# nmonette/TO-UED

Hardware: NVIDIA B200
Metric: gridworld agent env-steps/sec incl. LPG update (higher is better)
Workload: dtype f16/bf16 operands, f32 accumulate (GRU); f32 elsewhere

## Files before the change

include/toued.h:

```cpp
#ifndef TOUED_H
#define TOUED_H
#include <stdint.h>
#ifdef __cplusplus
extern "C" {
#endif

#define TOUED_LEVEL_BYTES 192

const char* toued_last_error(void);
int toued_version(void);

int toued_rollout(const void* levels, const uint32_t* keys, const float* actor,
                  const uint8_t* forced_actions, int32_t* state, int32_t* obs, uint8_t* action,
                  float* reward, uint8_t* done, float* ep_return, int n_agents, int n_workers,
                  int rollout_len, int obs_dim, int max_grid_size, int max_n_objs, int reset_first,
                  void* stream);

int toued_env_step(const void* levels, const uint32_t* keys, const int32_t* actions, int32_t* state,
                   int32_t* obs, float* reward, uint8_t* done, int n_agents, int n_workers,
                   int max_grid_size, int max_n_objs, void* stream);
int toued_env_reset(const void* levels, int32_t* state, int32_t* obs, int n_agents, int n_workers,
                    int max_grid_size, void* stream);


int toued_sort_tokens(const int32_t* obs, uint16_t* sorted_tok, int n_agents, int n_workers,
                      int rollout_len, void* stream);

int toued_lpg_prepare(const int32_t* obs, const uint8_t* action, const float* reward,
                      const uint8_t* done, const float* actor, const float* critic,
                      const float* lpg_params, const int32_t* step, const void* levels, float* x,
                      void* ximg, int n_agents, int n_workers, int rollout_len, int obs_dim,
                      int lifetime_conditioning, int lpg_stride, void* stream);

int toued_gru_forward(const float* x, const uint8_t* done, const float* lpg_params, float* h_out,
                      float* gates, float* pi_hat, float* y_hat, int n_agents, int n_workers,
                      int rollout_len, int lifetime_conditioning, int lpg_stride, void* stream);

int toued_agent_scratch_floats(int n_agents, int n_workers, int rollout_len, int obs_dim);
int toued_agent_update(const int32_t* obs, const uint8_t* action, const uint16_t* sorted_tok,
                       const float* pi_hat, const float* y_hat, const float* actor_in,
                       const float* critic_in, float* actor_out, float* critic_out,
                       const void* levels, int32_t* step, float* scalars, int n_agents,
                       int n_workers, int rollout_len, int obs_dim, float lr_actor, float lr_critic,
                       float max_grad_norm, float agent_target_coeff, int tables_precopied, float* run_scratch,
                       void* stream);


int toued_meta_loss(const int32_t* obs, const uint8_t* action, const float* reward,
                    const uint8_t* done, const uint16_t* sorted_tok, const float* value_table,
                    const float* actor, float* lam, float* mu, float* scalars, int n_agents,
                    int n_workers, int rollout_len, int obs_dim, int value_stride, float gamma,
                    float gae_lambda, float grad_scale, int outer_product_quirk, void* stream);

int toued_agent_backward(const int32_t* obs, const uint8_t* action, const uint16_t* sorted_tok,
                         const float* pi_hat, const float* y_hat, const float* actor_k,
                         const float* critic_k, const float* actor_k1, const float* critic_k1,
                         const float* update_scalars, float* lam, float* mu, float* d_pi_hat,
                         float* d_y_hat, int n_agents, int n_workers, int rollout_len, int obs_dim,
                         float lr_actor, float lr_critic, float max_grad_norm,
                         float agent_target_coeff, float policy_entropy_coeff,
                         float target_entropy_coeff, float policy_l2_coeff, float target_l2_coeff,
                         float grad_scale, float* run_scratch, void* stream);

int toued_transpose_wh(const float* lpg_params, float* whT, void* stream);

int toued_gru_backward(const uint8_t* done, const float* lpg_params, const float* whT,
                       const float* h, float* gates, const float* y_hat, const float* d_pi_hat,
                       const float* d_y_hat, float* dl, float* dx, int n_agents, int n_workers,
                       int rollout_len, int lifetime_conditioning, void* stream);

int toued_lpg_wgrad_workspace_floats(void);
int toued_lpg_wgrad(const int32_t* obs, const uint8_t* done, const float* critic,
                    const float* lpg_params, const float* x, const float* h, const float* dgates,
                    const float* d_pi_hat, const float* dl, const float* dx, float* workspace,
                    int n_agents, int n_workers, int rollout_len, int obs_dim,
                    int lifetime_conditioning, int accumulate, void* stream);
int toued_lpg_wgrad_workspace_offset(int which);
int toued_lpg_wgrad_embed(const int32_t* obs, const uint8_t* done, const float* critic, const float* lpg_params,
                          const float* dx, float* workspace, const uint32_t* cotangent_max, int n_agents, int n_workers,
                          int rollout_len, int obs_dim, int lifetime_conditioning, int accumulate, void* stream);
int toued_lpg_wgrad_splits(int which);
int toued_reduce_partials(const float* workspace, float* grad, int lifetime_conditioning, int wh_splits,
                          int sm_splits, void* stream);

int toued_adam(float* params, const float* grad, float* mu, float* nu, int n, int count, float lr,
               float b1, float b2, float eps, void* stream);
int toued_adam_dev(float* params, const float* grad, float* mu, float* nu, int* count_dev, int n, float lr,
                   float b1, float b2, float eps, void* stream);
int toued_sgd_clip(float* params, const float* grad, float* sqnorm_scratch, int n, float lr, float max_norm,
                   void* stream);

int toued_a2c_update(const int32_t* obs, const uint8_t* action, const float* reward, const uint8_t* done,
                     const uint16_t* sorted_tok, const float* actor_in, const float* critic_in,
                     float* actor_out, float* critic_out, const void* levels, int32_t* step,
                     float* scalars, int n_agents, int n_workers, int rollout_len, int obs_dim,
                     float lr_actor, float lr_critic, float max_grad_norm, float gamma, float gae_lambda,
                     float entropy_coeff, int outer_product_quirk, void* stream);

int toued_a2c_train(const void* levels, const uint32_t* keys, float* actor0, float* actor1, float* critic0,
                    float* critic1, int32_t* state, int32_t* obs, uint8_t* action, float* reward, uint8_t* done,
                    uint16_t* sorted_tok, int32_t* step, float* scalars, float* loss_sums, int num_updates,
                    int n_agents, int n_workers, int rollout_len, int obs_dim, int max_grid_size, int max_n_objs,
                    float lr_actor, float lr_critic, float max_grad_norm, float gamma, float gae_lambda,
                    float entropy_coeff, int outer_product_quirk, void* stream);

int toued_es_ask(const uint32_t* key, const float* mean, float sigma, float* candidates, int popsize,
                 int n_params, int cand_stride, void* stream);
int toued_es_tell(const float* candidates, const float* fitness, float* mean, float* m, float* v,
                  int popsize, int n_params, int cand_stride, float sigma, float lrate, float beta1,
                  float beta2, float eps, int gen_counter, float mean_decay, void* stream);

int toued_es_ask_shard(const uint32_t* key, const float* mean, float sigma, float* candidates, int popsize_global,
                       int n_params, int cand_stride, int pair_offset, int n_pairs, void* stream);
int toued_es_grad_partial(const float* candidates, const float* fitness, const float* mean, float* grad_sum,
                          int n_members, int n_params, int cand_stride, float sigma, void* stream);
int toued_es_adam(const float* grad_sum, float* mean, float* m, float* v, int popsize_global, int n_params,
                  float sigma, float lrate, float beta1, float beta2, float eps, int gen_counter, float mean_decay,
                  void* stream);

int toued_plr_reset_lowest(float* score, uint8_t* active, uint8_t* is_new, int buffer_size, int minimum_new,
                           int* reset_ids, void* stream);
int toued_plr_select(uint32_t key0, uint32_t key1, float* score, uint8_t* active, uint8_t* is_new, int buffer_size,
                     const int* old_ids, const uint8_t* terminated, const float* new_scores, int n_agents,
                     float p_replay, float temperature, int shuffle_rounds, int* new_ids, void* stream);

int toued_generate_levels_desc_bytes(void);
int toued_generate_levels(const void* gen_desc, const uint32_t* keys, const int32_t* buffer_ids, void* levels_out,
                          int32_t* lifetimes_out, int n_levels, void* stream);

int toued_optimal_return(const void* levels, int n_levels, int horizon, int max_grid_size, int max_n_objs,
                         double* out, void* stream);

int toued_get_nash(const float* game, const float* x0, const float* y0, float* x_out, float* y_out,
                   int n, int x_nz, int y_nz, int num_iters, float lr, void* stream);
int toued_projection_simplex(float* v, int n, int max_nz, void* stream);


int toued_init_tables(const uint32_t* keys, const uint8_t* mask, float* tables, int n_agents,
                      int obs_dim, int n_out, void* stream);
int toued_masked_reset(const void* levels, const uint8_t* mask, int32_t* state, int32_t* obs,
                       int32_t* step, int n_agents, int n_workers, int max_grid_size, void* stream);

int toued_host_iota_bits(const uint32_t* keys, int n_keys, int n, uint32_t* out);


int toued_key_split(const uint32_t* keys_in, int n_keys, int num, int offset, int count, uint32_t* out,
                    void* stream);
int toued_key_chain(const uint32_t* keys_in, int n_keys, int chain_len, uint32_t* keys_out,
                    uint32_t* carry_out, void* stream);


int toued_tc_gemm_test(const float* A, const float* B, void* scratch_img, float* D, void* stream);
int toued_tc_gemm_mixed_test(const float* A, const float* B, void* scratch_img, float* D, void* stream);
int toued_tc_gemm_mn_test(const float* A, const float* B, void* scratch_img, float* D, int lbo, int sbo,
                          int kadv, void* stream);
int toued_tc_gemm_mn2_test(const float* A, const float* B, void* scratch_img, float* D, void* stream);

int toued_pack_wh_forward(const float* lpg_params, void* wh_img, int lifetime_conditioning, void* stream);
int toued_gru_forward_tc(const float* x, const uint8_t* done, const float* lpg_params, const void* wh_img,
                         void* h16, void* fac, void* hpimg, float* pi_hat, float* y_hat, int n_agents,
                         int n_workers, int rollout_len, int lifetime_conditioning, void* stream);
int toued_pack_wh_forward_multi(const float* lpg_params, void* wh_img, int lifetime_conditioning, int n_sets,
                                int lpg_stride, void* stream);
int toued_gru_forward_tc_multi(const float* x, const uint8_t* done, const float* lpg_params, const void* wh_img,
                               float* pi_hat, float* y_hat, int n_agents, int n_workers, int rollout_len,
                               int lifetime_conditioning, int lpg_stride, void* stream);

int toued_pack_wh_backward(const float* lpg_params, void* whb_img, void* stream);
#define TOUED_STATUS_NONFINITE_COT 1u
#define TOUED_STATUS_FP16_RANGE 2u
int toued_cotangent_max(const float* d_pi_hat, const float* d_y_hat, int n_agents, int n_workers, int rollout_len,
                        uint32_t* cotangent_max, void* stream);
int toued_gru_backward_tc(const uint8_t* done, const float* lpg_params, const void* whb_img,
                          const void* h16, const void* fac, const float* y_hat, const float* d_pi_hat,
                          const float* d_y_hat, void* dgimg, float* dl, float* dx, uint32_t* cotangent_max,
                          int n_agents, int n_workers, int rollout_len, int lifetime_conditioning, void* stream);
int toued_wgrad_tc_splits(void);
int toued_wgrad_tc_small_splits(void);
int toued_lpg_wgrad_tc(const void* hpimg, const void* dgimg, const void* ximg, const void* h16,
                       const float* d_pi_hat, const float* dl, float* wh_partials, float* small_partials,
                       uint32_t* cotangent_max, int n_agents, int n_workers, int rollout_len, int accumulate,
                       void* stream);

#ifdef __cplusplus
}
#endif
#endif
```

to_ued_b200/_lib.py:

```python
from __future__ import annotations

import ctypes as C
import os

_HERE = os.path.dirname(os.path.abspath(__file__))
_VARIANT = os.environ.get("TOUED_LIB_VARIANT", "")
LIB_PATH = os.path.join(_HERE, f"libtoued_{_VARIANT}.so" if _VARIANT else "libtoued.so")

_lib = None


class TouedError(RuntimeError):
    pass


def lib() -> C.CDLL:
    global _lib
    if _lib is None:
        if not os.path.exists(LIB_PATH):
            raise TouedError(
                f"{LIB_PATH} is missing: the CUDA extension is not built. "
                "Run `python -m to_ued_b200.csrc.build` (there is no CPU fallback).")
        _lib = C.CDLL(LIB_PATH)
        _declare(_lib)
    return _lib


_P, _I, _F = C.c_void_p, C.c_int, C.c_float

SIGNATURES = {
    "toued_rollout": [_P] * 10 + [_I] * 7 + [_P],
    "toued_env_step": [_P] * 7 + [_I] * 4 + [_P],
    "toued_env_reset": [_P] * 3 + [_I] * 3 + [_P],
    "toued_sort_tokens": [_P] * 2 + [_I] * 3 + [_P],
    "toued_lpg_prepare": [_P] * 11 + [_I] * 6 + [_P],
    "toued_gru_forward": [_P] * 7 + [_I] * 5 + [_P],
    "toued_agent_update": [_P] * 12 + [_I] * 4 + [_F] * 4 + [_I, _P, _P],
    "toued_agent_scratch_floats": [_I] * 4,
    "toued_meta_loss": [_P] * 10 + [_I] * 5 + [_F] * 3 + [_I, _P],
    "toued_agent_backward": [_P] * 14 + [_I] * 4 + [_F] * 9 + [_P, _P],
    "toued_transpose_wh": [_P] * 3,
    "toued_gru_backward": [_P] * 10 + [_I] * 4 + [_P],
    "toued_lpg_wgrad_workspace_floats": [],
    "toued_lpg_wgrad": [_P] * 11 + [_I] * 6 + [_P],
    "toued_reduce_partials": [_P, _P, _I, _I, _I, _P],
    "toued_lpg_wgrad_splits": [_I],
    "toued_lpg_wgrad_workspace_offset": [_I],
    "toued_lpg_wgrad_embed": [_P] * 7 + [_I] * 6 + [_P],
    "toued_cotangent_max": [_P, _P, _I, _I, _I, _P, _P],
    "toued_pack_wh_backward": [_P] * 3,
    "toued_gru_backward_tc": [_P] * 12 + [_I] * 4 + [_P],
    "toued_wgrad_tc_splits": [],
    "toued_wgrad_tc_small_splits": [],
    "toued_lpg_wgrad_tc": [_P] * 9 + [_I] * 4 + [_P],
    "toued_adam": [_P] * 4 + [_I, _I] + [_F] * 4 + [_P],
    "toued_adam_dev": [_P] * 5 + [_I] + [_F] * 4 + [_P],
    "toued_sgd_clip": [_P] * 3 + [_I, _F, _F, _P],
    "toued_get_nash": [_P] * 5 + [_I] * 4 + [_F, _P],
    "toued_projection_simplex": [_P, _I, _I, _P],
    "toued_es_ask": [_P, _P, _F, _P, _I, _I, _I, _P],
    "toued_es_tell": [_P] * 5 + [_I, _I, _I] + [_F] * 5 + [_I, _F, _P],
    "toued_es_ask_shard": [_P, _P, _F, _P, _I, _I, _I, _I, _I, _P],
    "toued_es_grad_partial": [_P] * 4 + [_I, _I, _I, _F, _P],
    "toued_es_adam": [_P] * 4 + [_I, _I] + [_F] * 5 + [_I, _F, _P],
    "toued_a2c_update": [_P] * 12 + [_I] * 4 + [_F] * 6 + [_I, _P],
    "toued_a2c_train": [_P] * 15 + [_I] * 7 + [_F] * 6 + [_I, _P],
    "toued_init_tables": [_P] * 3 + [_I] * 3 + [_P],
    "toued_masked_reset": [_P] * 5 + [_I] * 3 + [_P],
    "toued_generate_levels_desc_bytes": [],
    "toued_generate_levels": [_P] * 5 + [_I, _P],
    "toued_plr_reset_lowest": [_P] * 3 + [_I, _I, _P, _P],
    "toued_plr_select": [C.c_uint32, C.c_uint32] + [_P] * 3 + [_I] + [_P] * 3 + [_I, _F, _F, _I, _P, _P],
    "toued_tc_gemm_test": [_P] * 5,
    "toued_tc_gemm_mixed_test": [_P] * 5,
    "toued_tc_gemm_mn_test": [_P] * 4 + [_I] * 3 + [_P],
    "toued_tc_gemm_mn2_test": [_P] * 5,
    "toued_pack_wh_forward": [_P, _P, _I, _P],
    "toued_pack_wh_forward_multi": [_P, _P, _I, _I, _I, _P],
    "toued_gru_forward_tc_multi": [_P] * 6 + [_I] * 5 + [_P],
    "toued_host_iota_bits": [_P, _I, _I, _P],
    "toued_key_split": [_P, _I, _I, _I, _I, _P, _P],
    "toued_key_chain": [_P, _I, _I, _P, _P, _P],
    "toued_gru_forward_tc": [_P] * 9 + [_I] * 4 + [_P],
    "toued_optimal_return": [_P] + [_I] * 4 + [_P, _P],
}


def _declare(l):
    l.toued_last_error.restype = C.c_char_p
    l.toued_last_error.argtypes = []
    l.toued_version.restype = _I
    l.toued_version.argtypes = []
    for name, args in SIGNATURES.items():
        fn = getattr(l, name)
        fn.restype = _I
        fn.argtypes = args


def ptr(t):
    if t is None:
        return None
    if not t.is_cuda:
        raise TouedError("to_ued_b200 ops need CUDA tensors (there is no CPU fallback)")
    if not t.is_contiguous():
        raise TouedError("to_ued_b200 ops need contiguous tensors")
    return t.data_ptr()


def stream_ptr():
    import torch
    return torch.cuda.current_stream().cuda_stream


KERNELS_PER_CALL = {"toued_adam_dev": 2, "toued_sgd_clip": 2, "toued_lpg_wgrad": 3, "toued_init_tables": 2, "toued_lpg_wgrad_tc": 2, "toued_pack_wh_forward": 2, "toued_pack_wh_forward_multi": 2}
LAUNCHES = {}
GRAPH_KERNELS = [0]
ENV_STEPS = [0]
PROFILE = None


H2D_BYTES = [0]


def h2d(t):
    H2D_BYTES[0] += int(t.numel() * t.element_size()) if hasattr(t, "element_size") else int(t.nbytes)
    return t


def reset_counters(profile=False):
    global PROFILE
    H2D_BYTES[0] = 0
    GRAPH_KERNELS[0] = 0
    ENV_STEPS[0] = 0
    LAUNCHES.clear()
    PROFILE = {} if profile else None


def kernel_launches():
    return sum(n * KERNELS_PER_CALL.get(k, 1) for k, n in LAUNCHES.items()) + GRAPH_KERNELS[0]


def profile_ms():
    return {k: (len(v), sum(a.elapsed_time(b) for a, b in v)) for k, v in (PROFILE or {}).items()}


def call(name, *args):
    LAUNCHES[name] = LAUNCHES.get(name, 0) + 1
    if name == "toued_rollout":
        ENV_STEPS[0] += args[10] * args[11] * args[12]
    elif name == "toued_a2c_train":
        ENV_STEPS[0] += args[15] * args[16] * args[17] * args[18]
    if PROFILE is not None:
        import torch
        a, b = torch.cuda.Event(enable_timing=True), torch.cuda.Event(enable_timing=True)
        a.record()
        rc = getattr(lib(), name)(*args)
        b.record()
        PROFILE.setdefault(name, []).append((a, b))
    else:
        rc = getattr(lib(), name)(*args)
    if rc != 0:
        raise TouedError(f"{name} failed ({rc}): {lib().toued_last_error().decode()}")
```

to_ued_b200/agents/lpg_agent.py:

```python
from __future__ import annotations

from dataclasses import dataclass, field
from typing import Any, List, Optional

import numpy as np
import torch

from .. import _lib
from ..util import prng
from ..util.data import AgentState, Transition


@dataclass
class LPGAgentMetrics:
    policy_l2: Any
    policy_entropy: Any
    critic_loss: Any
    critic_l2: Any
    critic_entropy: Any

    def as_dict(self):
        return {"policy_l2": self.policy_l2, "policy_entropy": self.policy_entropy,
                "critic_loss": self.critic_loss, "critic_l2": self.critic_l2,
                "critic_entropy": self.critic_entropy}


class Tape:

    def __init__(self, n_agents, n_workers, rollout_len, obs_dim, num_updates, device, keep_gates=True,
                 precision=None, per_agent_params=False):
        import to_ued_b200
        N, W, L, D, K = n_agents, n_workers, rollout_len, obs_dim, num_updates
        R, dev = N * W, device
        f32, u8, i32 = torch.float32, torch.uint8, torch.int32
        self.N, self.W, self.L, self.D, self.K, self.R = N, W, L, D, K, R
        self.record = bool(keep_gates)
        kt = K + 1 if self.record else 2
        kr = K + 1 if self.record else 1
        ka = K if self.record else 1
        self.kt, self.kr, self.ka = kt, kr, ka
        self.actor = torch.empty((kt, N, D, 8), dtype=f32, device=dev)
        self.critic = torch.empty((kt, N, D, 8), dtype=f32, device=dev)
        self.obs = torch.empty((kr, N, L + 1, W), dtype=i32, device=dev)
        self.action = torch.empty((kr, N, L, W), dtype=u8, device=dev)
        self.reward = torch.empty((kr, N, L, W), dtype=f32, device=dev)
        self.done = torch.empty((kr, N, L, W), dtype=u8, device=dev)
        self.sorted_tok = torch.empty((kr, N, L * W), dtype=torch.int16, device=dev)
        self.precision = precision or to_ued_b200.GRU_PRECISION
        self.x = torch.empty((ka, L, R, 8), dtype=f32, device=dev)
        self.ximg = None
        if self.precision == "tc":
            f16 = torch.float16
            Rp = (R + 63) // 64 * 64
            R32 = (R + 31) // 32 * 32
            self.h16 = torch.empty((ka, L, R32, 256), dtype=f16, device=dev) if self.record and not per_agent_params else None
            self.fac = torch.empty((ka, 4, L, R32, 256), dtype=f16, device=dev) if self.record else None
            self.hpimg = torch.zeros((ka, L * Rp * 256 * 2), dtype=torch.uint8, device=dev) if self.record else None
            self.ximg = torch.zeros((ka, L * Rp * 128), dtype=torch.uint8, device=dev) if self.record else None
            self.wh_img = torch.zeros((N if per_agent_params else 1) * 16 * 26624 // 2, dtype=f16, device=dev)
            self.h = self.gates = None
        else:
            self.h = torch.empty((ka, L, R, 256), dtype=f32, device=dev)
            self.gates = torch.empty((ka, 4, L, R, 256), dtype=f32, device=dev) if self.record else None
        self.pi_hat = torch.empty((ka, L, R), dtype=f32, device=dev)
        self.y_hat = torch.empty((ka, L, R, 8), dtype=f32, device=dev)
        self.scalars = torch.empty((ka, N, 8), dtype=f32, device=dev)
        self.scal_sum = torch.zeros((N, 8), dtype=f32, device=dev)
        self.step_in = torch.empty((ka, N), dtype=i32, device=dev)
        self.ep_return = torch.empty((N, W), dtype=f32, device=dev)
        self.agent_scratch = torch.empty(_lib.lib().toued_agent_scratch_floats(N, W, L, D), dtype=f32, device=dev)

    def ti(self, k):
        return k if self.record else (k & 1)

    def ri(self, k):
        return k if self.record else 0

    def ai(self, k):
        return k if self.record else 0

    def transition(self, k) -> Transition:
        r = self.ri(k)
        return Transition(self.obs[r], self.action[r], self.reward[r], self.done[r])


_SORT_STREAMS = {}


def _sort_stream(cur):
    key = (cur.device.index, cur.cuda_stream)
    st = _SORT_STREAMS.get(key)
    if st is None:
        st = _SORT_STREAMS[key] = torch.cuda.Stream(device=cur.device)
    return st


def _mark(label):
    import to_ued_b200
    if to_ued_b200.PHASE_EVENTS is not None and getattr(to_ued_b200, "PHASE_FINE", False):
        e = torch.cuda.Event(enable_timing=True)
        e.record(torch.cuda.current_stream())
        to_ued_b200.PHASE_EVENTS.append((label, -2, e))


def lpg_agent_train_step(k, tape: Tape, levels, step, lpg_params, lifetime_conditioning, agent_target_coeff,
                         lr_actor, lr_critic, max_grad_norm, lpg_stride=0):
    N, W, L, D = tape.N, tape.W, tape.L, tape.D
    s = _lib.stream_ptr()
    p = _lib.ptr
    r, a, t0, t1 = tape.ri(k), tape.ai(k), tape.ti(k), tape.ti(k + 1)
    import to_ued_b200
    cur = torch.cuda.current_stream()
    side = _sort_stream(cur) if to_ued_b200.SIDE_STREAMS else cur
    ev_roll, ev_sort = torch.cuda.Event(), torch.cuda.Event()
    ev_roll.record(cur)
    with torch.cuda.stream(side):
        side.wait_event(ev_roll)
        _lib.call("toued_sort_tokens", p(tape.obs[r]), p(tape.sorted_tok[r]), N, W, L, _lib.stream_ptr())
        precopied = bool(to_ued_b200.SIDE_STREAMS)
        if precopied:
            tape.actor[t1].copy_(tape.actor[t0])
            tape.critic[t1].copy_(tape.critic[t0])
        ev_sort.record(side)
    _mark("rollout")
    tape.step_in[a].copy_(step)
    _lib.call("toued_lpg_prepare", p(tape.obs[r]), p(tape.action[r]), p(tape.reward[r]), p(tape.done[r]),
              p(tape.actor[t0]), p(tape.critic[t0]), p(lpg_params), p(step), p(levels), p(tape.x[a]),
              p(tape.ximg[a]) if tape.ximg is not None else None,
              N, W, L, D, int(lifetime_conditioning), int(lpg_stride), s)
    if lpg_stride and tape.precision == "tc":
        _lib.call("toued_gru_forward_tc_multi", p(tape.x[a]), p(tape.done[r]), p(lpg_params), p(tape.wh_img),
                  p(tape.pi_hat[a]), p(tape.y_hat[a]), N, W, L, int(lifetime_conditioning), int(lpg_stride), s)
    elif lpg_stride or tape.precision != "tc":
        _lib.call("toued_gru_forward", p(tape.x[a]), p(tape.done[r]), p(lpg_params), p(tape.h[a]),
                  p(tape.gates[a]) if tape.gates is not None else None, p(tape.pi_hat[a]), p(tape.y_hat[a]),
                  N, W, L, int(lifetime_conditioning), int(lpg_stride), s)
    else:
        _lib.call("toued_gru_forward_tc", p(tape.x[a]), p(tape.done[r]), p(lpg_params), p(tape.wh_img),
                  p(tape.h16[a]) if tape.h16 is not None else None, p(tape.fac[a]) if tape.fac is not None else None,
                  p(tape.hpimg[a]) if tape.hpimg is not None else None, p(tape.pi_hat[a]), p(tape.y_hat[a]),
                  N, W, L, int(lifetime_conditioning), s)
    _mark("gru_fwd")
    cur.wait_event(ev_sort)
    _mark("sort_wait")
    _lib.call("toued_agent_update", p(tape.obs[r]), p(tape.action[r]), p(tape.sorted_tok[r]), p(tape.pi_hat[a]),
              p(tape.y_hat[a]), p(tape.actor[t0]), p(tape.critic[t0]), p(tape.actor[t1]), p(tape.critic[t1]),
              p(levels), p(step), p(tape.scalars[a]), N, W, L, D, float(lr_actor), float(lr_critic),
              float(max_grad_norm), float(agent_target_coeff), int(precopied), p(tape.agent_scratch), s)
    tape.scal_sum += tape.scalars[a]
    _mark("update")


def train_lpg_agent_steps(rng, lpg_train_state, agent_state: AgentState, rollout_manager, num_train_steps: int,
                          agent_target_coeff: float, tape: Optional[Tape] = None, lpg_stride: int = 0):
    env = rollout_manager.env
    actor, critic = agent_state.actor_state, agent_state.critic_state
    N, W = agent_state.env_state.packed.shape
    L, K = rollout_manager.train_rollout_len, num_train_steps
    dev = actor.params.device
    if tape is None:
        import to_ued_b200
        tape = Tape(N, W, L, env.obs_dim, K, dev, keep_gates=False,
                    precision=to_ued_b200.ES_PRECISION if lpg_stride else None, per_agent_params=bool(lpg_stride))
    levels = agent_state.level.packed
    step = actor.step.clone()
    state = agent_state.env_state.packed.clone()
    tape.actor[0].copy_(actor.params)
    tape.critic[0].copy_(critic.params)
    tape.scal_sum.zero_()
    keys_d = prng.chain_device(prng.to_device(rng, dev), K)
    p = _lib.ptr
    lpg = lpg_train_state.params if hasattr(lpg_train_state, "params") else lpg_train_state
    cond = lpg_train_state.model.lifetime_conditioning if hasattr(lpg_train_state, "model") else False
    if tape.precision == "tc" and not lpg_stride:
        _lib.call("toued_pack_wh_forward", p(lpg), p(tape.wh_img), int(cond), _lib.stream_ptr())
    elif tape.precision == "tc":
        _lib.call("toued_pack_wh_forward_multi", p(lpg), p(tape.wh_img), int(cond), N, int(lpg_stride), _lib.stream_ptr())
    yield
    for k in range(K):
        r = tape.ri(k)
        _lib.call("toued_rollout", p(levels), p(keys_d[k]), p(tape.actor[tape.ti(k)]), None, p(state), p(tape.obs[r]),
                  p(tape.action[r]), p(tape.reward[r]), p(tape.done[r]), None, N, W, L, env.obs_dim,
                  env.max_grid_size, env.max_n_objs, 0, _lib.stream_ptr())
        lpg_agent_train_step(k, tape, levels, step, lpg, cond, agent_target_coeff, actor.learning_rate,
                             critic.learning_rate, actor.max_grad_norm, lpg_stride=lpg_stride)
        yield
    sc = tape.scal_sum / K
    metrics = LPGAgentMetrics(policy_l2=sc[:, 4], policy_entropy=sc[:, 6], critic_loss=sc[:, 3],
                              critic_l2=sc[:, 5], critic_entropy=sc[:, 7])
    from ..environments.gridworld.gridworld import EnvState
    new_agent = agent_state.replace(
        actor_state=actor.replace(params=tape.actor[tape.ti(K)].clone(), step=step),
        critic_state=critic.replace(params=tape.critic[tape.ti(K)].clone(), step=step.clone()),
        env_obs=tape.obs[tape.ri(K - 1)][:, -1].clone(), env_state=EnvState(state, env.max_n_objs))
    rollouts = [tape.transition(k) for k in range(K)] if tape.record else [tape.transition(K - 1)]
    return new_agent, rollouts, metrics


def train_lpg_agent(rng, lpg_train_state, agent_state: AgentState, rollout_manager, num_train_steps: int,
                    agent_target_coeff: float, tape: Optional[Tape] = None, lpg_stride: int = 0):
    gen = train_lpg_agent_steps(rng, lpg_train_state, agent_state, rollout_manager, num_train_steps,
                                agent_target_coeff, tape=tape, lpg_stride=lpg_stride)
    while True:
        try:
            next(gen)
        except StopIteration as done:
            return done.value
```

to_ued_b200/csrc/agent_backward.cu:

```cuda
#include "lpg_common.cuh"
#include "segreduce.cuh"
#include "../../include/toued.h"

__global__ void __launch_bounds__(256)
meta_loss_kernel(const int32_t* __restrict__ obs, const uint8_t* __restrict__ action,
                 const float* __restrict__ reward, const uint8_t* __restrict__ done,
                 const uint16_t* __restrict__ sorted_tok, const float* __restrict__ value,
                 const float* __restrict__ actor, float* __restrict__ lam, float* __restrict__ mu,
                 float* __restrict__ scal, int W, int L, int D, int vstride, float gamma, float lmbda,
                 float gscale, int quirk) {
    extern __shared__ __align__(16) float sm[];
    float* adv = sm;
    float* rec = adv + L * W;
    float* abar = rec + L * W * 6;
    float* lbar = abar + W;
    float* runv = lbar + W;
    float* scan = runv + L * W * 5;
    void* idxmem = scan + 2 * 256 * 5;
    __shared__ float red[32];
    __shared__ int iscan[512];
    __shared__ unsigned char sflags[512];
    const int n = blockIdx.x, tid = threadIdx.x, T = W * L;
    const int32_t* ob = obs + (size_t)n * (L + 1) * W;
    const uint8_t* act = action + (size_t)n * T;
    const float* rw = reward + (size_t)n * T;
    const uint8_t* dn = done + (size_t)n * T;
    const uint16_t* st = sorted_tok + (size_t)n * T;
    const float* vt = value + (size_t)n * D * vstride;
    const float* at = actor + (size_t)n * D * 8;
    float* lm = lam + (size_t)n * D * 8;
    float* mm = mu + (size_t)n * D * 8;
    const float invT = 1.0f / (float)T;
    const SegIndex si = seg_index_build(idxmem, iscan, st, ob, T);

    for (int i = tid; i < D * 2; i += 256) {
        reinterpret_cast<float4*>(lm)[i] = make_float4(0.f, 0.f, 0.f, 0.f);
        reinterpret_cast<float4*>(mm)[i] = make_float4(0.f, 0.f, 0.f, 0.f);
    }
    float s1 = 0.f, s2 = 0.f;
    const float vlast = vt[(size_t)(D - 1) * vstride];
    for (int w = tid; w < W; w += 256) {
        float g = 0.f;
        int32_t o1 = ob[L * W + w];
        float v1 = vt[(size_t)ob_idx(o1) * vstride] + 0.001f * (float)ob_time(o1) * vlast;
        for (int t = L - 1; t >= 0; --t) {
            const int32_t o0 = ob[t * W + w];
            const float v0 = vt[(size_t)ob_idx(o0) * vstride] + 0.001f * (float)ob_time(o0) * vlast;
            const float nd = dn[t * W + w] ? 0.0f : 1.0f;
            const float delta = rw[t * W + w] + gamma * v1 * nd - v0;
            g = delta + gamma * lmbda * nd * g;
            adv[t * W + w] = g;
            s1 += g; s2 = fmaf(g, g, s2);
            v1 = v0;
        }
    }
    s1 = block_sum(s1, red); s2 = block_sum(s2, red);
    const float mean = s1 * invT;
    float var = 0.f;
    for (int i = tid; i < T; i += 256) { const float d = adv[i] - mean; var = fmaf(d, d, var); }
    var = block_sum(var, red) * invT;
    const float inv_std = 1.0f / (sqrtf(var) + 1e-8f);
    __syncthreads();
    for (int i = tid; i < T; i += 256) adv[i] = (adv[i] - mean) * inv_std;
    __syncthreads();
    for (int tok = tid; tok < T; tok += 256) {
        const int32_t o = ob[tok];
        float z[5], p[5];
        tab_logits8<5>(at, D, o, z);
        softmax_c<5>(z, p);
        const int a = act[tok];
        float pa = p[0];
#pragma unroll
        for (int j = 1; j < 5; ++j) pa = (a == j) ? p[j] : pa;
        float* r = rec + tok * 6;
        r[5] = logf(pa + 1e-8f);
        const float q = pa / (pa + 1e-8f);
#pragma unroll
        for (int j = 0; j < 5; ++j) r[j] = q * ((a == j ? 1.0f : 0.0f) - p[j]);
    }
    __syncthreads();
    float loss = 0.f;
    for (int w = tid; w < W; w += 256) {
        float sa = 0.f, sl = 0.f, se = 0.f;
        for (int t = 0; t < L; ++t) { sa += adv[t * W + w]; sl += rec[(t * W + w) * 6 + 5]; se = fmaf(adv[t * W + w], rec[(t * W + w) * 6 + 5], se); }
        abar[w] = sa / (float)L; lbar[w] = sl / (float)L;
        loss -= quirk ? abar[w] * lbar[w] : se / (float)L;
    }
    loss = block_sum(loss, red) / (float)W;
    __syncthreads();
    float last[5] = {0.f, 0.f, 0.f, 0.f, 0.f};
    for (int tok = tid; tok < T; tok += 256) {
        const int w = tok % W;
        const float coef = -gscale * invT * (quirk ? abar[w] : adv[tok]);
        float* r = rec + tok * 6;
        const float tf = 0.001f * (float)ob_time(ob[tok]);
#pragma unroll
        for (int j = 0; j < 5; ++j) { r[j] *= coef; last[j] = fmaf(tf, r[j], last[j]); }
        r[5] = tf;
    }
#pragma unroll
    for (int j = 0; j < 5; ++j) last[j] = block_sum(last[j], red);
    __syncthreads();
    seg_reduce<5, 6>(rec, si, T, runv, scan, sflags);
    for (int r = tid; r < si.nruns; r += 256) {
        const int row = si.run_row[r];
#pragma unroll
        for (int j = 0; j < 5; ++j) lm[(size_t)row * 8 + j] = runv[r * 5 + j];
    }
    if (tid == 0) {
#pragma unroll
        for (int j = 0; j < 5; ++j) lm[(size_t)(D - 1) * 8 + j] = last[j];
        scal[n * 2 + 0] = loss;
        scal[n * 2 + 1] = s2 * invT;
    }
}

extern "C" int toued_meta_loss(const int32_t* obs, const uint8_t* action, const float* reward,
                               const uint8_t* done, const uint16_t* sorted_tok, const float* value_table,
                               const float* actor, float* lam, float* mu, float* scalars, int n_agents,
                               int n_workers, int rollout_len, int obs_dim, int value_stride, float gamma,
                               float gae_lambda, float grad_scale, int outer_product_quirk, void* stream) {
    const int T = n_workers * rollout_len;
    TOUED_CHECK(n_agents > 0 && T > 0, "toued_meta_loss: empty problem");
    const size_t smem = sizeof(float) * ((size_t)T * 7 + 2 * n_workers + (size_t)T * 5 + 2 * 256 * 5) + seg_index_bytes(T);
    TOUED_CHECK(smem <= 200 * 1024, "toued_meta_loss: W*L=%d too large for shared memory", T);
    TOUED_CUDA(cudaFuncSetAttribute(meta_loss_kernel, cudaFuncAttributeMaxDynamicSharedMemorySize, (int)smem));
    meta_loss_kernel<<<n_agents, 256, smem, (cudaStream_t)stream>>>(
        obs, action, reward, done, sorted_tok, value_table, actor, lam, mu, scalars, n_workers, rollout_len,
        obs_dim, value_stride, gamma, gae_lambda, grad_scale, outer_product_quirk);
    TOUED_LAUNCH_CHECK();
    return 0;
}

struct TokFwd { float p[5], y[8], pa, q, tf; int a; };

__device__ __forceinline__ TokFwd tok_forward(const float* at, const float* ct, int D, int32_t o, int a) {
    TokFwd f;
    float z[5], zy[8];
    tab_logits8<5>(at, D, o, z);
    softmax_c<5>(z, f.p);
    tab_logits8<8>(ct, D, o, zy);
    softmax_c<8>(zy, f.y);
    f.a = a;
    f.pa = f.p[0];
#pragma unroll
    for (int j = 1; j < 5; ++j) f.pa = (a == j) ? f.p[j] : f.pa;
    f.q = f.pa / (f.pa + 1e-8f);
    f.tf = 0.001f * (float)ob_time(o);
    return f;
}

__device__ __forceinline__ void tok_grad(const TokFwd& f, float ph, const float* yh, float invT, float alpha, float* c) {
    const float ca = invT * ph * f.q;
#pragma unroll
    for (int j = 0; j < 5; ++j) c[j] = ca * ((f.a == j ? 1.0f : 0.0f) - f.p[j]);
    float mm[8], b = 0.f;
#pragma unroll
    for (int i = 0; i < 8; ++i) {
        mm[i] = logf(f.y[i] + 1e-8f) - logf(yh[i] + 1e-8f) + f.y[i] / (f.y[i] + 1e-8f);
        b = fmaf(f.y[i], mm[i], b);
    }
    const float cc = alpha * invT;
#pragma unroll
    for (int i = 0; i < 8; ++i) c[5 + i] = cc * f.y[i] * (mm[i] - b);
}

__device__ __forceinline__ void load8(const float* p, float* v) {
    const float4 a = reinterpret_cast<const float4*>(p)[0], b = reinterpret_cast<const float4*>(p)[1];
    v[0] = a.x; v[1] = a.y; v[2] = a.z; v[3] = a.w; v[4] = b.x; v[5] = b.y; v[6] = b.z; v[7] = b.w;
}

__global__ void __launch_bounds__(256, 2)
agent_backward_kernel(const int32_t* __restrict__ obs, const uint8_t* __restrict__ action,
                      const uint16_t* __restrict__ sorted_tok, const float* __restrict__ pi_hat,
                      const float* __restrict__ y_hat, const float* __restrict__ actor_k,
                      const float* __restrict__ critic_k, const float* __restrict__ actor_k1,
                      const float* __restrict__ critic_k1, const float* __restrict__ upd_scal,
                      float* lam, float* mu, float* __restrict__ d_pi_hat, float* __restrict__ d_y_hat,
                      float* run_scratch, int n_agents, int W, int L, int D, float lr_a, float lr_c, float max_norm,
                      float alpha, float b_pent, float b_yent, float b_pl2, float b_yl2, float gscale) {
    extern __shared__ __align__(16) float rec[];
    __shared__ float red[32];
    __shared__ float s_wlast[13];
    __shared__ int iscan[512];
    __shared__ unsigned char sflags[512];
    const int n = blockIdx.x, tid = threadIdx.x, T = W * L, R = n_agents * W;
    const int32_t* ob = obs + (size_t)n * (L + 1) * W;
    const uint8_t* act = action + (size_t)n * T;
    const uint16_t* st = sorted_tok + (size_t)n * T;
    const float* a0 = actor_k + (size_t)n * D * 8;
    const float* c0 = critic_k + (size_t)n * D * 8;
    const float* a1 = actor_k1 + (size_t)n * D * 8;
    const float* c1 = critic_k1 + (size_t)n * D * 8;
    float* lm = lam + (size_t)n * D * 8;
    float* mm = mu + (size_t)n * D * 8;
    const float invT = 1.0f / (float)T;
    const float gna = upd_scal[n * 8 + 0], gnc = upd_scal[n * 8 + 1];
    const bool keep = upd_scal[n * 8 + 2] != 0.0f;
    float* runv = run_scratch + (size_t)n * min(T, D) * 13;
    float* scan = rec + (size_t)T * 13;
    const SegIndex si = seg_index_build(scan + 2 * 256 * 13, iscan, st, ob, T);

    float last[13];
#pragma unroll
    for (int j = 0; j < 13; ++j) last[j] = 0.f;
    for (int tok = tid; tok < T; tok += 256) {
        const TokFwd f = tok_forward(a1, c1, D, ob[tok], act[tok]);
        float* r = rec + tok * 13;
        {
            float dh[5], s = 0.f;
#pragma unroll
            for (int j = 0; j < 5; ++j) { dh[j] = -(logf(f.p[j] + 1e-8f) + 1.0f); s = fmaf(f.p[j], dh[j], s); }
            const float k = -b_pent * gscale * invT;
#pragma unroll
            for (int j = 0; j < 5; ++j) r[j] = k * f.p[j] * (dh[j] - s);
        }
        {
            float dh[8], s = 0.f;
#pragma unroll
            for (int j = 0; j < 8; ++j) { dh[j] = -(logf(f.y[j] + 1e-8f) + 1.0f); s = fmaf(f.y[j], dh[j], s); }
            const float k = -b_yent * gscale * invT;
#pragma unroll
            for (int j = 0; j < 8; ++j) r[5 + j] = k * f.y[j] * (dh[j] - s);
        }
#pragma unroll
        for (int j = 0; j < 13; ++j) last[j] = fmaf(f.tf, r[j], last[j]);
    }
#pragma unroll
    for (int j = 0; j < 13; ++j) last[j] = block_sum(last[j], red);
    __syncthreads();
    seg_reduce<13, 13>(rec, si, T, runv, scan, sflags);
    for (int r = tid; r < si.nruns; r += 256) {
        const int row = si.run_row[r];
        const float* g = runv + r * 13;
#pragma unroll
        for (int j = 0; j < 5; ++j) lm[(size_t)row * 8 + j] += g[j];
#pragma unroll
        for (int j = 0; j < 8; ++j) mm[(size_t)row * 8 + j] += g[5 + j];
    }
    if (tid == 0) {
#pragma unroll
        for (int j = 0; j < 5; ++j) lm[(size_t)(D - 1) * 8 + j] += last[j];
#pragma unroll
        for (int j = 0; j < 8; ++j) mm[(size_t)(D - 1) * 8 + j] += last[5 + j];
    }
    __syncthreads();

    const float dir_pi = gscale * b_pl2 * 2.0f * invT;
    const float dir_y = gscale * b_yl2 * 2.0f * invT;
    if (!keep) {
        for (int tok = tid; tok < T; tok += 256) {
            const int t = tok / W, w = tok - t * W;
            const size_t li = (size_t)t * R + (size_t)n * W + w;
            d_pi_hat[li] = dir_pi * pi_hat[li];
            float yh[8]; load8(y_hat + li * 8, yh);
            float4* o = reinterpret_cast<float4*>(d_y_hat + li * 8);
            o[0] = make_float4(dir_y * yh[0], dir_y * yh[1], dir_y * yh[2], dir_y * yh[3]);
            o[1] = make_float4(dir_y * yh[4], dir_y * yh[5], dir_y * yh[6], dir_y * yh[7]);
        }
        return;
    }

#pragma unroll
    for (int j = 0; j < 13; ++j) last[j] = 0.f;
    for (int tok = tid; tok < T; tok += 256) {
        const int t = tok / W, w = tok - t * W;
        const size_t li = (size_t)t * R + (size_t)n * W + w;
        const TokFwd f = tok_forward(a0, c0, D, ob[tok], act[tok]);
        float yh[8]; load8(y_hat + li * 8, yh);
        float* r = rec + tok * 13;
        tok_grad(f, pi_hat[li], yh, invT, alpha, r);
#pragma unroll
        for (int j = 0; j < 13; ++j) last[j] = fmaf(f.tf, r[j], last[j]);
    }
#pragma unroll
    for (int j = 0; j < 13; ++j) last[j] = block_sum(last[j], red);
    __syncthreads();
    seg_reduce<13, 13>(rec, si, T, runv, scan, sflags);
    float dot_a = 0.f, dot_c = 0.f;
    for (int r = tid; r < si.nruns; r += 256) {
        const int row = si.run_row[r];
        const float* g = runv + r * 13;
        float l8[8], m8[8];
        load8(lm + (size_t)row * 8, l8); load8(mm + (size_t)row * 8, m8);
#pragma unroll
        for (int j = 0; j < 5; ++j) dot_a = fmaf(g[j], l8[j], dot_a);
#pragma unroll
        for (int j = 0; j < 8; ++j) dot_c = fmaf(g[5 + j], m8[j], dot_c);
    }
    dot_a = block_sum(dot_a, red); dot_c = block_sum(dot_c, red);
    float ll[8], ml[8];
    load8(lm + (size_t)(D - 1) * 8, ll); load8(mm + (size_t)(D - 1) * 8, ml);
#pragma unroll
    for (int j = 0; j < 5; ++j) dot_a = fmaf(last[j], ll[j], dot_a);
#pragma unroll
    for (int j = 0; j < 8; ++j) dot_c = fmaf(last[5 + j], ml[j], dot_c);
    const bool clip_a = !(gna < max_norm), clip_c = !(gnc < max_norm);
    const float ka = -lr_a * (clip_a ? max_norm / gna : 1.0f), pa_ = clip_a ? dot_a / (gna * gna) : 0.0f;
    const float kc = -lr_c * (clip_c ? max_norm / gnc : 1.0f), pc_ = clip_c ? dot_c / (gnc * gnc) : 0.0f;
    if (tid == 0) {
#pragma unroll
        for (int j = 0; j < 5; ++j) s_wlast[j] = ka * (ll[j] - pa_ * last[j]);
#pragma unroll
        for (int j = 0; j < 8; ++j) s_wlast[5 + j] = kc * (ml[j] - pc_ * last[5 + j]);
    }
    __syncthreads();
    float wl[13];
#pragma unroll
    for (int j = 0; j < 13; ++j) wl[j] = s_wlast[j];

    for (int r = tid; r < si.nruns; r += 256) {
        const int row = si.run_row[r];
        float* g = runv + r * 13;
        float l8[8], m8[8];
        load8(lm + (size_t)row * 8, l8); load8(mm + (size_t)row * 8, m8);
#pragma unroll
        for (int j = 0; j < 5; ++j) g[j] = ka * (l8[j] - pa_ * g[j]);
#pragma unroll
        for (int j = 0; j < 8; ++j) g[5 + j] = kc * (m8[j] - pc_ * g[5 + j]);
    }
    __syncthreads();
    float hl[13];
#pragma unroll
    for (int j = 0; j < 13; ++j) hl[j] = 0.f;
    for (int pos = tid; pos < T; pos += 256) {
        const int tok = si.tok[pos];
        const int t = tok / W, w = tok - t * W;
        const size_t li = (size_t)t * R + (size_t)n * W + w;
        const TokFwd f = tok_forward(a0, c0, D, ob[tok], act[tok]);
        const float ph = pi_hat[li];
        float yh[8]; load8(y_hat + li * 8, yh);
        float* r = rec + tok * 13;
        const float* wr = runv + (size_t)si.run[pos] * 13;
        float v[13];
#pragma unroll
        for (int j = 0; j < 13; ++j) v[j] = fmaf(f.tf, wl[j], wr[j]);
        float va = v[0], pv = 0.f;
#pragma unroll
        for (int j = 1; j < 5; ++j) va = (f.a == j) ? v[j] : va;
#pragma unroll
        for (int j = 0; j < 5; ++j) pv = fmaf(f.p[j], v[j], pv);
        const float s = va - pv;
        d_pi_hat[li] = invT * f.q * s + dir_pi * ph;
        const float pe = f.pa + 1e-8f;
        const float c1_ = ph * invT * s * 1e-8f * f.pa / (pe * pe), c2_ = ph * invT * f.q;
        float h[13];
#pragma unroll
        for (int j = 0; j < 5; ++j)
            h[j] = c1_ * ((f.a == j ? 1.0f : 0.0f) - f.p[j]) - c2_ * f.p[j] * (v[j] - pv);
        float m[8], mp[8], av = 0.f, b = 0.f;
#pragma unroll
        for (int j = 0; j < 8; ++j) {
            const float ye = f.y[j] + 1e-8f;
            m[j] = logf(ye) - logf(yh[j] + 1e-8f) + f.y[j] / ye;
            mp[j] = (f.y[j] + 2e-8f) / (ye * ye);
            av = fmaf(v[5 + j], f.y[j], av);
            b = fmaf(f.y[j], m[j], b);
        }
        const float ca = alpha * invT;
        float dS[8], sy = 0.f, dyo[8];
#pragma unroll
        for (int j = 0; j < 8; ++j) {
            const float vc = v[5 + j];
            dyo[j] = ca * f.y[j] * (av - vc) / (yh[j] + 1e-8f) + dir_y * yh[j];
            dS[j] = vc * m[j] + vc * f.y[j] * mp[j] - vc * b - av * (m[j] + f.y[j] * mp[j]);
            sy = fmaf(f.y[j], dS[j], sy);
        }
#pragma unroll
        for (int j = 0; j < 8; ++j) h[5 + j] = ca * f.y[j] * (dS[j] - sy);
        float4* o = reinterpret_cast<float4*>(d_y_hat + li * 8);
        o[0] = make_float4(dyo[0], dyo[1], dyo[2], dyo[3]);
        o[1] = make_float4(dyo[4], dyo[5], dyo[6], dyo[7]);
#pragma unroll
        for (int j = 0; j < 13; ++j) { r[j] = h[j]; hl[j] = fmaf(f.tf, h[j], hl[j]); }
    }
#pragma unroll
    for (int j = 0; j < 13; ++j) hl[j] = block_sum(hl[j], red);
    __syncthreads();
    seg_reduce<13, 13>(rec, si, T, runv, scan, sflags);
    for (int r = tid; r < si.nruns; r += 256) {
        const int row = si.run_row[r];
        const float* g = runv + r * 13;
#pragma unroll
        for (int j = 0; j < 5; ++j) lm[(size_t)row * 8 + j] += g[j];
#pragma unroll
        for (int j = 0; j < 8; ++j) mm[(size_t)row * 8 + j] += g[5 + j];
    }
    if (tid == 0) {
#pragma unroll
        for (int j = 0; j < 5; ++j) lm[(size_t)(D - 1) * 8 + j] = ll[j] + hl[j];
#pragma unroll
        for (int j = 0; j < 8; ++j) mm[(size_t)(D - 1) * 8 + j] = ml[j] + hl[5 + j];
    }
}

extern "C" int toued_agent_backward(const int32_t* obs, const uint8_t* action, const uint16_t* sorted_tok,
                                    const float* pi_hat, const float* y_hat, const float* actor_k,
                                    const float* critic_k, const float* actor_k1, const float* critic_k1,
                                    const float* update_scalars, float* lam, float* mu, float* d_pi_hat,
                                    float* d_y_hat, int n_agents, int n_workers, int rollout_len, int obs_dim,
                                    float lr_actor, float lr_critic, float max_grad_norm,
                                    float agent_target_coeff, float policy_entropy_coeff,
                                    float target_entropy_coeff, float policy_l2_coeff, float target_l2_coeff,
                                    float grad_scale, float* run_scratch, void* stream) {
    const int T = n_workers * rollout_len;
    TOUED_CHECK(n_agents > 0 && T > 0, "toued_agent_backward: empty problem");
    TOUED_CHECK(run_scratch != nullptr, "toued_agent_backward: run_scratch (toued_agent_scratch_floats) is required");
    const size_t smem = sizeof(float) * ((size_t)T * 13 + 2 * 256 * 13) + seg_index_bytes(T);
    TOUED_CHECK(smem <= 200 * 1024, "toued_agent_backward: W*L=%d too large for shared memory", T);
    TOUED_CUDA(cudaFuncSetAttribute(agent_backward_kernel, cudaFuncAttributeMaxDynamicSharedMemorySize, (int)smem));
    TOUED_CUDA(cudaFuncSetAttribute(agent_backward_kernel, cudaFuncAttributePreferredSharedMemoryCarveout, 100));
    cudaStream_t st = (cudaStream_t)stream;
    agent_backward_kernel<<<n_agents, 256, smem, st>>>(
        obs, action, sorted_tok, pi_hat, y_hat, actor_k, critic_k, actor_k1, critic_k1, update_scalars, lam, mu,
        d_pi_hat, d_y_hat, run_scratch, n_agents, n_workers, rollout_len, obs_dim, lr_actor, lr_critic, max_grad_norm,
        agent_target_coeff, policy_entropy_coeff, target_entropy_coeff, policy_l2_coeff, target_l2_coeff, grad_scale);
    TOUED_LAUNCH_CHECK();
    return 0;
}
```

to_ued_b200/csrc/agent_update.cu:

```cuda
#include "lpg_common.cuh"
#include "segreduce.cuh"
#include "../../include/toued.h"

constexpr int AU_C = 13;

__global__ void __launch_bounds__(256, 2)
agent_update_kernel(const int32_t* __restrict__ obs, const uint8_t* __restrict__ action,
                    const uint16_t* __restrict__ sorted_tok, const float* __restrict__ pi_hat,
                    const float* __restrict__ y_hat, const float* __restrict__ actor_in,
                    const float* __restrict__ critic_in, float* actor_out, float* critic_out,
                    const LevelRec* __restrict__ levels, int32_t* __restrict__ step,
                    float* __restrict__ scal, float* run_scratch, int n_agents, int W, int L, int D,
                    float lr_a, float lr_c, float max_norm, float alpha, int tables_precopied) {
    extern __shared__ __align__(16) float smc[];
    __shared__ float red[32];
    __shared__ int iscan[512];
    __shared__ unsigned char sflags[512];
    const int n = blockIdx.x, tid = threadIdx.x, T = W * L, R = n_agents * W;
    float* runv = run_scratch + (size_t)n * min(T, D) * 13;
    float* scan = smc + (size_t)T * AU_C;
    void* idxmem = scan + 2 * 256 * 13;
    const int32_t* ob = obs + (size_t)n * (L + 1) * W;
    const uint8_t* act = action + (size_t)n * T;
    const float* a_in = actor_in + (size_t)n * D * 8;
    const float* c_in = critic_in + (size_t)n * D * 8;
    float* a_out = actor_out + (size_t)n * D * 8;
    float* c_out = critic_out + (size_t)n * D * 8;
    const float invT = 1.0f / (float)T;
    const SegIndex si = seg_index_build(idxmem, iscan, sorted_tok + (size_t)n * T, ob, T);

    if (!tables_precopied)
        for (int i = tid; i < D * 2; i += 256) {
            reinterpret_cast<float4*>(a_out)[i] = reinterpret_cast<const float4*>(a_in)[i];
            reinterpret_cast<float4*>(c_out)[i] = reinterpret_cast<const float4*>(c_in)[i];
        }

    float m_kl = 0.f, m_pi2 = 0.f, m_y2 = 0.f;
    float last[13];
#pragma unroll
    for (int j = 0; j < 13; ++j) last[j] = 0.f;
    for (int tok = tid; tok < T; tok += 256) {
        const int t = tok / W, w = tok - t * W;
        const size_t li = (size_t)t * R + (size_t)n * W + w;
        const int32_t o = ob[tok];
        float z[5], p[5], zy[8], y[8];
        tab_logits8<5>(a_in, D, o, z);
        softmax_c<5>(z, p);
        tab_logits8<8>(c_in, D, o, zy);
        softmax_c<8>(zy, y);
        const int a = act[tok];
        float pa = p[0];
#pragma unroll
        for (int j = 1; j < 5; ++j) pa = (a == j) ? p[j] : pa;
        const float ph = pi_hat[li];
        const float ca = invT * ph * (pa / (pa + 1e-8f));
        float* rec = smc + tok * AU_C;
#pragma unroll
        for (int j = 0; j < 5; ++j) rec[j] = ca * ((a == j ? 1.0f : 0.0f) - p[j]);
        float yh[8];
        { const float4* q = reinterpret_cast<const float4*>(y_hat + li * 8); const float4 q0 = q[0], q1 = q[1];
          yh[0] = q0.x; yh[1] = q0.y; yh[2] = q0.z; yh[3] = q0.w; yh[4] = q1.x; yh[5] = q1.y; yh[6] = q1.z; yh[7] = q1.w; }
        float mm[8], b = 0.f, kl = 0.f, y2 = 0.f;
#pragma unroll
        for (int i = 0; i < 8; ++i) {
            const float ly = logf(y[i] + 1e-8f), lh = logf(yh[i] + 1e-8f);
            mm[i] = ly - lh + y[i] / (y[i] + 1e-8f);
            b = fmaf(y[i], mm[i], b);
            kl = fmaf(y[i], ly - lh, kl);
            y2 = fmaf(yh[i], yh[i], y2);
        }
        const float cc = alpha * invT;
#pragma unroll
        for (int i = 0; i < 8; ++i) rec[5 + i] = cc * y[i] * (mm[i] - b);
        const float tf = 0.001f * (float)ob_time(o);
#pragma unroll
        for (int j = 0; j < 13; ++j) last[j] = fmaf(tf, rec[j], last[j]);
        m_kl += kl; m_pi2 = fmaf(ph, ph, m_pi2); m_y2 += y2;
    }
#pragma unroll
    for (int j = 0; j < 13; ++j) last[j] = block_sum(last[j], red);
    m_kl = block_sum(m_kl, red); m_pi2 = block_sum(m_pi2, red); m_y2 = block_sum(m_y2, red);
    __syncthreads();

    seg_reduce<13, AU_C>(smc, si, T, runv, scan, sflags);
    float na = 0.f, nc = 0.f;
    for (int r = tid; r < si.nruns; r += 256) {
        const float* g = runv + r * 13;
#pragma unroll
        for (int j = 0; j < 5; ++j) na = fmaf(g[j], g[j], na);
#pragma unroll
        for (int j = 5; j < 13; ++j) nc = fmaf(g[j], g[j], nc);
    }
    na = block_sum(na, red); nc = block_sum(nc, red);
#pragma unroll
    for (int j = 0; j < 5; ++j) na = fmaf(last[j], last[j], na);
#pragma unroll
    for (int j = 5; j < 13; ++j) nc = fmaf(last[j], last[j], nc);
    const float gna = sqrtf(na), gnc = sqrtf(nc);
    const float sa = gna < max_norm ? 1.0f : max_norm / gna;
    const float sc = gnc < max_norm ? 1.0f : max_norm / gnc;
    const int old_step = step[n];
    const bool keep = (old_step + 1) <= levels[n].lifetime;
    const float ua = keep ? lr_a * sa : 0.0f, uc = keep ? lr_c * sc : 0.0f;

    for (int r = tid; r < si.nruns; r += 256) {
        const int row = si.run_row[r];
        const float* g = runv + r * 13;
#pragma unroll
        for (int j = 0; j < 5; ++j) a_out[(size_t)row * 8 + j] = a_in[(size_t)row * 8 + j] - ua * g[j];
#pragma unroll
        for (int j = 0; j < 8; ++j) c_out[(size_t)row * 8 + j] = c_in[(size_t)row * 8 + j] - uc * g[5 + j];
    }
    if (tid == 0) {
#pragma unroll
        for (int j = 0; j < 5; ++j) a_out[(size_t)(D - 1) * 8 + j] = a_in[(size_t)(D - 1) * 8 + j] - ua * last[j];
#pragma unroll
        for (int j = 0; j < 8; ++j) c_out[(size_t)(D - 1) * 8 + j] = c_in[(size_t)(D - 1) * 8 + j] - uc * last[5 + j];
        step[n] = keep ? old_step + 1 : old_step;
    }
    __syncthreads();

    float ea = 0.f, ec = 0.f;
    for (int tok = tid; tok < T; tok += 256) {
        const int32_t o = ob[tok];
        float z[5], p[5], zy[8], y[8];
        tab_logits8<5>(a_out, D, o, z);
        softmax_c<5>(z, p);
        tab_logits8<8>(c_out, D, o, zy);
        softmax_c<8>(zy, y);
#pragma unroll
        for (int j = 0; j < 5; ++j) { const float q = p[j] + 1e-8f; ea -= q * logf(q); }
#pragma unroll
        for (int j = 0; j < 8; ++j) { const float q = y[j] + 1e-8f; ec -= q * logf(q); }
    }
    ea = block_sum(ea, red); ec = block_sum(ec, red);
    if (tid == 0) {
        float* s = scal + (size_t)n * 8;
        s[0] = gna; s[1] = gnc; s[2] = keep ? 1.0f : 0.0f;
        s[3] = m_kl * invT;
        s[4] = m_pi2 * invT;
        s[5] = m_y2 * invT;
        s[6] = ea * invT;
        s[7] = ec * invT;
    }
}

static size_t agent_smem_bytes(int T, int D) {
    return sizeof(float) * ((size_t)T * AU_C + 2 * 256 * 13) + seg_index_bytes(T);
}

extern "C" int toued_agent_update(const int32_t* obs, const uint8_t* action, const uint16_t* sorted_tok,
                                  const float* pi_hat, const float* y_hat, const float* actor_in,
                                  const float* critic_in, float* actor_out, float* critic_out,
                                  const void* levels, int32_t* step, float* scalars, int n_agents,
                                  int n_workers, int rollout_len, int obs_dim, float lr_actor,
                                  float lr_critic, float max_grad_norm, float agent_target_coeff, int tables_precopied,
                                  float* run_scratch, void* stream) {
    const int T = n_workers * rollout_len;
    const size_t smem = agent_smem_bytes(T, obs_dim);
    TOUED_CHECK(n_agents > 0 && T > 0, "toued_agent_update: empty problem");
    TOUED_CHECK(smem <= 200 * 1024, "toued_agent_update: W*L=%d too large for shared memory", T);
    TOUED_CHECK(actor_in != actor_out && critic_in != critic_out, "toued_agent_update: in-place update not supported");
    TOUED_CUDA(cudaFuncSetAttribute(agent_update_kernel, cudaFuncAttributeMaxDynamicSharedMemorySize, (int)smem));
    TOUED_CUDA(cudaFuncSetAttribute(agent_update_kernel, cudaFuncAttributePreferredSharedMemoryCarveout, 100));
    TOUED_CHECK(run_scratch != nullptr, "toued_agent_update: run_scratch (toued_agent_scratch_floats) is required");
    cudaStream_t st = (cudaStream_t)stream;
    agent_update_kernel<<<n_agents, 256, smem, st>>>(
        obs, action, sorted_tok, pi_hat, y_hat, actor_in, critic_in, actor_out, critic_out,
        (const LevelRec*)levels, step, scalars, run_scratch, n_agents, n_workers, rollout_len, obs_dim,
        lr_actor, lr_critic, max_grad_norm, agent_target_coeff, tables_precopied);
    TOUED_LAUNCH_CHECK();
    return 0;
}

extern "C" int toued_agent_scratch_floats(int n_agents, int n_workers, int rollout_len, int obs_dim) {
    const long long T = (long long)n_workers * rollout_len;
    const long long n = 13ll * (T < obs_dim ? T : obs_dim) * n_agents;
    return n < (1ll << 31) ? (int)n : -1;
}
```

to_ued_b200/csrc/lpg_common.cuh:

```cuda
#pragma once
#include "common.cuh"

constexpr int LPG_H = 256;
constexpr int LPG_Y = 8;
constexpr int LPG_E = 16;
constexpr int LPG_G = 3 * LPG_H;
constexpr int LPG_XP = 8;

struct LpgOffsets {
    int e_w0, e_b0, e_w1, e_b1, Wi, bi, Wh, bhn, w_pi, b_pi, W_y, b_y, total;
};
__host__ __device__ inline LpgOffsets lpg_offsets(int X) {
    LpgOffsets o; int p = 0;
    o.Wh = p; p += LPG_H * LPG_G;
    o.Wi = p; p += X * LPG_G;
    o.bi = p; p += LPG_G;
    o.bhn = p; p += LPG_H;
    o.w_pi = p; p += LPG_H;
    o.W_y = p; p += LPG_H * LPG_Y;
    o.b_y = p; p += LPG_Y;
    o.e_w0 = p; p += LPG_Y * LPG_E;
    o.e_b0 = p; p += LPG_E;
    o.e_w1 = p; p += LPG_E;
    o.e_b1 = p; p += 1;
    o.b_pi = p; p += 1;
    o.total = p;
    return o;
}

__device__ __forceinline__ float sigmoidf_(float x) { return 1.0f / (1.0f + __expf(-x)); }
__device__ __forceinline__ float tanhf_(float x) {
    const float e = __expf(2.0f * x);
    return 1.0f - 2.0f / (e + 1.0f);
}

__device__ __forceinline__ float ex2_approx(float x) { float y; asm("ex2.approx.ftz.f32 %0, %1;" : "=f"(y) : "f"(x)); return y; }
__device__ __forceinline__ float rcp_approx(float x) { float y; asm("rcp.approx.ftz.f32 %0, %1;" : "=f"(y) : "f"(x)); return y; }
__device__ __forceinline__ float tanh_mufu(float x) { float y; asm("tanh.approx.f32 %0, %1;" : "=f"(y) : "f"(x)); return y; }
__device__ __forceinline__ float sigmoid_mufu(float x) { return fmaf(0.5f, tanh_mufu(0.5f * x), 0.5f); }
__device__ __forceinline__ float sigmoid_fast(float x) { return rcp_approx(1.0f + ex2_approx(-1.4426950408889634f * x)); }
__device__ __forceinline__ float tanh_fast(float x) { return fmaf(2.0f, rcp_approx(1.0f + ex2_approx(-2.8853900817779268f * x)), -1.0f); }

__device__ __forceinline__ float fmin_nan(float a, float b) { float r; asm("min.NaN.f32 %0, %1, %2;" : "=f"(r) : "f"(a), "f"(b)); return r; }
__device__ __forceinline__ float fmax_nan(float a, float b) { float r; asm("max.NaN.f32 %0, %1, %2;" : "=f"(r) : "f"(a), "f"(b)); return r; }
__device__ __forceinline__ float fmax3_nan(float a, float b, float c) {
    float r; asm("max.NaN.f32 %0, %1, %2, %3;" : "=f"(r) : "f"(a), "f"(b), "f"(c)); return r;
}

template <int C>
__device__ __forceinline__ void softmax_c(const float (&z)[C], float (&p)[C]) {
    float m = z[0];
#pragma unroll
    for (int j = 1; j < C; ++j) m = fmaxf(m, z[j]);
    float s = 0.0f;
#pragma unroll
    for (int j = 0; j < C; ++j) { p[j] = __expf(z[j] - m); s += p[j]; }
    const float inv = 1.0f / s;
#pragma unroll
    for (int j = 0; j < C; ++j) p[j] *= inv;
}

template <int C>
__device__ __forceinline__ void tab_logits8(const float* table, int D, int32_t ob, float (&z)[C]) {
    const float tf = 0.001f * (float)ob_time(ob);
    const float4* row = reinterpret_cast<const float4*>(table + (size_t)ob_idx(ob) * 8);
    const float4* last = reinterpret_cast<const float4*>(table + (size_t)(D - 1) * 8);
    float r[8], l[8];
    const float4 a0 = row[0], a1 = row[1], b0 = last[0], b1 = last[1];
    r[0] = a0.x; r[1] = a0.y; r[2] = a0.z; r[3] = a0.w; r[4] = a1.x; r[5] = a1.y; r[6] = a1.z; r[7] = a1.w;
    l[0] = b0.x; l[1] = b0.y; l[2] = b0.z; l[3] = b0.w; l[4] = b1.x; l[5] = b1.y; l[6] = b1.z; l[7] = b1.w;
#pragma unroll
    for (int j = 0; j < C; ++j) z[j] = r[j] + tf * l[j];
}

__device__ __forceinline__ float block_sum(float v, float* red) {
#pragma unroll
    for (int o = 16; o > 0; o >>= 1) v += __shfl_xor_sync(0xffffffffu, v, o);
    const int lane = threadIdx.x & 31, warp = threadIdx.x >> 5, nw = (blockDim.x + 31) >> 5;
    __syncthreads();
    if (lane == 0) red[warp] = v;
    __syncthreads();
    float t = (lane < nw) ? red[lane] : 0.0f;
#pragma unroll
    for (int o = 16; o > 0; o >>= 1) t += __shfl_xor_sync(0xffffffffu, t, o);
    return t;
}
```

to_ued_b200/meta/train.py:

```python
from __future__ import annotations

from typing import Any, Optional

import numpy as np
import torch

from .. import _lib
from ..util import prng
from ..util.data import AgentState, LpgHyperparams
from ..agents.lpg_agent import Tape, train_lpg_agent, train_lpg_agent_steps
from ..agents.agents import eval_agent
from ..environments.gridworld.gridworld import EnvState


class LPGTrainState:

    def __init__(self, model, params, tx, opt_state=None, step=0):
        self.model, self.params, self.tx = model, params, tx
        self.opt_state = tx.init(params) if opt_state is None else opt_state
        self.step = step

    def replace(self, **kw):
        d = dict(model=self.model, params=self.params, tx=self.tx, opt_state=self.opt_state, step=self.step)
        d.update(kw)
        return LPGTrainState(**d)


class MetaGradWorkspace:

    def __init__(self, n_agents, n_workers, rollout_len, obs_dim, num_updates, n_params, device):
        N, W, L, K = n_agents, n_workers, rollout_len, num_updates
        R = N * W
        f32 = torch.float32
        self.tape = Tape(N, W, L, obs_dim, K, device, keep_gates=True)
        self.d_pi_hat2 = [torch.empty((L, R), dtype=f32, device=device) for _ in range(2)]
        self.d_y_hat2 = [torch.empty((L, R, 8), dtype=f32, device=device) for _ in range(2)]
        self.dx2 = [torch.empty((L, R, 2), dtype=f32, device=device) for _ in range(2)]
        self.d_pi_hat, self.d_y_hat, self.dx = self.d_pi_hat2[0], self.d_y_hat2[0], self.dx2[0]
        self.dl2 = [torch.empty((L, R, 8), dtype=f32, device=device) for _ in range(2)]
        self.dl = self.dl2[0]
        self.lam = torch.empty((N, obs_dim, 8), dtype=f32, device=device)
        self.mu = torch.empty((N, obs_dim, 8), dtype=f32, device=device)
        self.whT = torch.empty((768, 256), dtype=f32, device=device)
        self.partials = torch.empty(_lib.lib().toued_lpg_wgrad_workspace_floats(), dtype=f32, device=device)
        self.loss_scal = torch.empty((N, 2), dtype=f32, device=device)
        self.ab_scratch = torch.empty(_lib.lib().toued_agent_scratch_floats(N, W, L, obs_dim), dtype=f32, device=device)
        if self.tape.precision == "tc":
            Rp = (R + 63) // 64 * 64
            self.whb_img = torch.empty(256 * 768, dtype=torch.float16, device=device)
            self.cotmax = torch.zeros((K, 2), dtype=torch.int32, device=device)
            self.dgimg2 = [torch.zeros(L * Rp * 1024 * 2, dtype=torch.uint8, device=device) for _ in range(2)]
            self.dgimg = self.dgimg2[0]
        self.off_small = _lib.lib().toued_lpg_wgrad_workspace_offset(1)
        self.key = (N, W, L, obs_dim, K, n_params, str(device))


_WS_CACHE = {}
_STREAMS = {}


def _workspace(n, w, L, D, K, P, device, slot=0) -> MetaGradWorkspace:
    import to_ued_b200
    key = (n, w, L, D, K, P, str(device), to_ued_b200.GRU_PRECISION)
    if _WS_CACHE and next(iter(_WS_CACHE))[:-1] != key:
        _WS_CACHE.clear()
    ws = _WS_CACHE.get(key + (slot,))
    if ws is None:
        ws = _WS_CACHE[key + (slot,)] = MetaGradWorkspace(n, w, L, D, K, P, device)
    return ws


def reverse_status(reset=False):
    st = torch.zeros((), dtype=torch.int32, device="cuda")
    for ws in _WS_CACHE.values():
        if getattr(ws, "cotmax", None) is not None:
            for w in ws.cotmax[:, 1]:
                st = st | w
            if reset:
                ws.cotmax[:, 1].zero_()
    return st


def _eval_stream(device):
    key = ("eval", str(device))
    if key not in _STREAMS:
        _STREAMS[key] = [torch.cuda.Stream(device=device)]
    return _STREAMS[key][0]


def _side_streams(device, n):
    key = str(device)
    lst = _STREAMS.setdefault(key, [])
    while len(lst) < n:
        lst.append(torch.cuda.Stream(device=device))
    return lst[:n]


def _world():
    import torch.distributed as dist
    if dist.is_available() and dist.is_initialized():
        return dist.get_world_size(), dist
    return 1, None


def lpg_meta_grad_train_step(rng, lpg_train_state: LPGTrainState, agent_states: AgentState, value_critic_states,
                             rollout_manager, num_mini_batches: int, gamma: float, gae_lambda: float,
                             lpg_hypers: LpgHyperparams, *, outer_product_quirk: bool = True,
                             global_agent_offset: int = 0, global_num_agents: Optional[int] = None,
                             eval_workers: int = 4, return_grad: bool = False, num_streams: Optional[int] = None,
                             _static: Optional[dict] = None):
    env = rollout_manager.env
    actor, critic = agent_states.actor_state, agent_states.critic_state
    N, W = agent_states.env_state.packed.shape
    L, K, D = rollout_manager.train_rollout_len, lpg_hypers.num_agent_updates, env.obs_dim
    dev = actor.params.device
    world, dist = _world()
    n_global = global_num_agents if global_num_agents is not None else N * world
    if dist is not None and global_num_agents is None:
        global_agent_offset = dist.get_rank() * N
    model = lpg_train_state.model
    cond = int(model.lifetime_conditioning)
    lpg = lpg_train_state.params
    P = lpg.numel()
    p, s = _lib.ptr, _lib.stream_ptr()

    rngs = prng.split_device(prng.to_device(rng, dev), n_global, global_agent_offset, N)[0]
    r_train, r_eval, r_evalagent = prng.chain_device(rngs, 3)

    if N % num_mini_batches != 0:
        raise ValueError(f"local agents ({N}) must be divisible by num_mini_batches ({num_mini_batches})")
    nb = N // num_mini_batches
    import to_ued_b200
    if num_streams is None:
        num_streams = to_ued_b200.NUM_STREAMS
    S = max(1, min(int(num_streams), num_mini_batches))
    wss = [_workspace(nb, W, L, D, K, P, dev, slot=i) for i in range(S)]
    main = torch.cuda.current_stream()
    streams = [main] if S == 1 else _side_streams(dev, S)
    tc = wss[0].tape.precision == "tc"
    gscale = 1.0 / n_global
    bK = [c / K for c in (lpg_hypers.policy_entropy_coeff, lpg_hypers.target_entropy_coeff,
                          lpg_hypers.policy_l2_coeff, lpg_hypers.target_l2_coeff)]
    if _static is not None:
        new_actor, new_critic, new_step, new_state, new_obs = _static["out"]
    else:
        new_actor = torch.empty_like(actor.params)
        new_critic = torch.empty_like(critic.params)
        new_step = torch.empty_like(actor.step)
        new_state = torch.empty_like(agent_states.env_state.packed)
        new_obs = torch.empty_like(agent_states.env_obs)
    msums = [torch.zeros(8, dtype=torch.float32, device=dev) for _ in range(S)]
    returns = torch.empty(N, dtype=torch.float32, device=dev)
    ready = torch.cuda.Event()
    ready.record(main)

    def _phase(label, chunk, stream):
        if to_ued_b200.PHASE_EVENTS is not None:
            e = torch.cuda.Event(enable_timing=True)
            e.record(stream)
            to_ued_b200.PHASE_EVENTS.append((label, chunk, e))
    _phase("start", -1, main)
    eval_done = [None] * S
    eval_stream = _side_streams(dev, S + 1)[S] if S > 1 else _eval_stream(dev)
    pool = _side_streams(dev, 5 * S + 1)
    ab_streams, em_streams = pool[S + 1:2 * S + 1], pool[2 * S + 1:3 * S + 1]
    ev_streams = [eval_stream] + pool[3 * S + 1:4 * S]
    wg_streams = pool[4 * S + 1:5 * S + 1]
    if not to_ued_b200.SIDE_STREAMS:
        ab_streams = em_streams = ev_streams = wg_streams = list(streams)
    evs = {}

    ctx, gens = {}, {}

    def forward_begin(mb):
        slot = mb % S
        ws, tape = wss[slot], wss[slot].tape
        with torch.cuda.stream(streams[slot]):
            if S > 1 and mb < S:
                streams[slot].wait_event(ready)
            if eval_done[slot] is not None:
                streams[slot].wait_event(eval_done[slot])
            sl = slice(mb * nb, (mb + 1) * nb)
            sub = AgentState(actor.replace(params=actor.params[sl], step=actor.step[sl]),
                             critic.replace(params=critic.params[sl], step=critic.step[sl]),
                             _sub_level(agent_states.level, sl), agent_states.env_obs[sl],
                             EnvState(agent_states.env_state.packed[sl], env.max_n_objs))
            levels = sub.level.packed
            gens[mb] = (train_lpg_agent_steps(r_train[sl], lpg_train_state, sub, rollout_manager, K,
                                              lpg_hypers.agent_target_coeff, tape=tape), sl, levels)
            next(gens[mb][0])

    def forward_step(mb):
        with torch.cuda.stream(streams[mb % S]):
            try:
                next(gens[mb][0])
            except StopIteration as fin:
                gens[mb] = (fin.value,) + gens[mb][1:]
            _phase("update", mb, streams[mb % S])

    def forward_end(mb):
        slot = mb % S
        ws, tape = wss[slot], wss[slot].tape
        res, sl, levels = gens.pop(mb)
        with torch.cuda.stream(streams[slot]):
            s = _lib.stream_ptr()
            if not isinstance(res, tuple):
                try:
                    while True:
                        next(res)
                except StopIteration as fin:
                    res = fin.value
            sub2, _, am = res
            state = sub2.env_state.packed
            _lib.call("toued_rollout", p(levels), p(r_eval[sl]), p(tape.actor[K]), None, p(state), p(tape.obs[K]),
                      p(tape.action[K]), p(tape.reward[K]), p(tape.done[K]), None, nb, W, L, D,
                      env.max_grid_size, env.max_n_objs, 0, s)
            _lib.call("toued_sort_tokens", p(tape.obs[K]), p(tape.sorted_tok[K]), nb, W, L, s)
            fwd_done = torch.cuda.Event()
            fwd_done.record(streams[slot])
            _phase("forward", mb, streams[slot])
            with torch.cuda.stream(ev_streams[slot]):
                ev_streams[slot].wait_event(fwd_done)
                returns[sl] = eval_agent(r_evalagent[sl], rollout_manager, levels, tape.actor[K], eval_workers)
                eval_done[slot] = torch.cuda.Event()
                eval_done[slot].record(ev_streams[slot])
            ctx[mb] = (sl, sub2, state, am, levels)

    def backward_begin(mb):
        slot = mb % S
        ws, tape = wss[slot], wss[slot].tape
        sl = ctx[mb][0]
        with torch.cuda.stream(streams[slot]):
            s = _lib.stream_ptr()
            if mb < S:
                if tc:
                    _lib.call("toued_pack_wh_backward", p(lpg), p(ws.whb_img), s)
                else:
                    _lib.call("toued_transpose_wh", p(lpg), p(ws.whT), s)
            vparams = value_critic_states.params[sl]
            _lib.call("toued_meta_loss", p(tape.obs[K]), p(tape.action[K]), p(tape.reward[K]), p(tape.done[K]),
                      p(tape.sorted_tok[K]), p(vparams), p(tape.actor[K]), p(ws.lam), p(ws.mu), p(ws.loss_scal),
                      nb, W, L, D, vparams.shape[-1], float(gamma), float(gae_lambda), float(gscale),
                      int(outer_product_quirk), s)
            evs[mb] = {"ml": torch.cuda.Event(), "ab": {}, "bwd": {}, "wg": {}, "em": {}}
            evs[mb]["ml"].record(streams[slot])

    def _agent_backward(ws, tape, k, buf, s):
        _lib.call("toued_agent_backward", p(tape.obs[k]), p(tape.action[k]), p(tape.sorted_tok[k]),
                  p(tape.pi_hat[k]), p(tape.y_hat[k]), p(tape.actor[k]), p(tape.critic[k]),
                  p(tape.actor[k + 1]), p(tape.critic[k + 1]), p(tape.scalars[k]), p(ws.lam), p(ws.mu),
                  p(ws.d_pi_hat2[buf]), p(ws.d_y_hat2[buf]), nb, W, L, D, float(actor.learning_rate),
                  float(critic.learning_rate), float(actor.max_grad_norm),
                  float(lpg_hypers.agent_target_coeff), *[float(b) for b in bK], float(gscale), p(ws.ab_scratch), s)

    def backward_step(mb, k):
        slot = mb % S
        ws, tape = wss[slot], wss[slot].tape
        first = (mb < S and k == K - 1)
        if not tc:
            with torch.cuda.stream(streams[slot]):
                s = _lib.stream_ptr()
                _agent_backward(ws, tape, k, 0, s)
                _lib.call("toued_gru_backward", p(tape.done[k]), p(lpg), p(ws.whT), p(tape.h[k]), p(tape.gates[k]),
                          p(tape.y_hat[k]), p(ws.d_pi_hat), p(ws.d_y_hat), p(ws.dl), p(ws.dx), nb, W, L, cond, s)
                _lib.call("toued_lpg_wgrad", p(tape.obs[k]), p(tape.done[k]), p(tape.critic[k]), p(lpg), p(tape.x[k]),
                          p(tape.h[k]), p(tape.gates[k]), p(ws.d_pi_hat), p(ws.dl), p(ws.dx), p(ws.partials),
                          nb, W, L, D, cond, 0 if first else 1, s)
            return
        ev, buf = evs[mb], k & 1
        for d in ("ab", "bwd", "wg", "em"):
            ev[d][k] = torch.cuda.Event()
        with torch.cuda.stream(ab_streams[slot]):
            st = ab_streams[slot]
            if k == K - 1:
                st.wait_event(ev["ml"])
            if k + 2 <= K - 1:
                st.wait_event(ev["wg"][k + 2])
            _agent_backward(ws, tape, k, buf, _lib.stream_ptr())
            _lib.call("toued_cotangent_max", p(ws.d_pi_hat2[buf]), p(ws.d_y_hat2[buf]), nb, W, L, p(ws.cotmax[k]),
                      _lib.stream_ptr())
            ev["ab"][k].record(st)
        with torch.cuda.stream(streams[slot]):
            st = streams[slot]
            s = _lib.stream_ptr()
            st.wait_event(ev["ab"][k])
            if k + 2 <= K - 1:
                st.wait_event(ev["em"][k + 2])
                st.wait_event(ev["wg"][k + 2])
            _lib.call("toued_gru_backward_tc", p(tape.done[k]), p(lpg), p(ws.whb_img), p(tape.h16[k]),
                      p(tape.fac[k]), p(tape.y_hat[k]), p(ws.d_pi_hat2[buf]), p(ws.d_y_hat2[buf]), p(ws.dgimg2[buf]), p(ws.dl2[buf]),
                      p(ws.dx2[buf]), p(ws.cotmax[k]), nb, W, L, cond, s)
            ev["bwd"][k].record(st)
            _phase(f"bwd{k}", mb, st)
        with torch.cuda.stream(wg_streams[slot]):
            st = wg_streams[slot]
            st.wait_event(ev["bwd"][k])
            _lib.call("toued_lpg_wgrad_tc", p(tape.hpimg[k]), p(ws.dgimg2[buf]), p(tape.ximg[k]), p(tape.h16[k]),
                      p(ws.d_pi_hat2[buf]), p(ws.dl2[buf]), p(ws.partials), p(ws.partials[ws.off_small:]),
                      p(ws.cotmax[k]), nb, W, L, 0 if first else 1, _lib.stream_ptr())
            ev["wg"][k].record(st)
            _phase(f"wgrad{k}", mb, st)
        with torch.cuda.stream(em_streams[slot]):
            st = em_streams[slot]
            st.wait_event(ev["bwd"][k])
            _lib.call("toued_lpg_wgrad_embed", p(tape.obs[k]), p(tape.done[k]), p(tape.critic[k]), p(lpg),
                      p(ws.dx2[buf]), p(ws.partials), p(ws.cotmax[k]), nb, W, L, D, cond, 0 if first else 1,
                      _lib.stream_ptr())
            ev["em"][k].record(st)

    def backward_end(mb):
        slot = mb % S
        ws, tape, msum = wss[slot], wss[slot].tape, msums[slot]
        sl, sub2, state, am, levels = ctx.pop(mb)
        with torch.cuda.stream(streams[slot]):
            ev = evs.pop(mb)
            if ev["em"]:
                streams[slot].wait_event(ev["em"][0])
                streams[slot].wait_event(ev["wg"][0])
            lpg_loss, value_loss = ws.loss_scal[:, 0], ws.loss_scal[:, 1]
            reg = (lpg_loss - lpg_hypers.policy_entropy_coeff * am.policy_entropy + lpg_hypers.policy_l2_coeff * am.policy_l2
                   - lpg_hypers.target_entropy_coeff * am.critic_entropy + lpg_hypers.target_l2_coeff * am.critic_l2)
            msum[:7] += torch.stack([lpg_loss.sum(), reg.sum(), value_loss.sum(), am.policy_l2.sum(),
                                     am.policy_entropy.sum(), am.critic_loss.sum(), am.critic_l2.sum()])
            msum[7] += am.critic_entropy.sum()
            new_actor[sl] = sub2.actor_state.params
            new_critic[sl] = sub2.critic_state.params
            new_step[sl] = sub2.actor_state.step
            new_state[sl] = state
            new_obs[sl] = tape.obs[K][:, -1]
            _phase("reverse_end", mb, streams[slot])

    for g0 in range(0, num_mini_batches, S):
        group = range(g0, min(num_mini_batches, g0 + S))
        for mb in group:
            forward_begin(mb)
            forward_step(mb)
        for k in range(1, K):
            for mb in group:
                forward_step(mb)
        for mb in group:
            forward_end(mb)
        for mb in group:
            backward_begin(mb)
        for k in reversed(range(K)):
            for mb in group:
                backward_step(mb, k)
        for mb in group:
            backward_end(mb)
    for st in ([] if S == 1 else list(streams)) + ev_streams:
        ev = torch.cuda.Event()
        ev.record(st)
        main.wait_event(ev)
    s = _lib.stream_ptr()
    msum = msums[0] if S == 1 else torch.stack(msums).sum(0)

    grad = torch.empty(P, dtype=torch.float32, device=dev)
    L_ = _lib.lib()
    n_wh, n_sm = (L_.toued_wgrad_tc_splits(), L_.toued_wgrad_tc_small_splits()) if tc else \
        (L_.toued_lpg_wgrad_splits(0), L_.toued_lpg_wgrad_splits(1))
    _lib.call("toued_reduce_partials", p(wss[0].partials), p(grad), cond, n_wh, n_sm, s)
    for ws in wss[1:min(S, num_mini_batches)]:
        g2 = torch.empty_like(grad)
        _lib.call("toued_reduce_partials", p(ws.partials), p(g2), cond, n_wh, n_sm, s)
        grad += g2
    red = torch.cat([grad, msum, returns.sum().view(1)])
    if dist is not None:
        dist.all_reduce(red)
    grad, mvec = red[:P], red[P:] / n_global
    if _static is not None:
        ost = lpg_train_state.opt_state
        lpg_train_state.tx.update_dev_(lpg, grad, ost["mu"], ost["nu"], _static["count_dev"])
        new_lpg = lpg_train_state
    else:
        new_params = lpg.clone()
        opt_state = lpg_train_state.tx.update_(new_params, grad, {**lpg_train_state.opt_state,
                                                                  "mu": lpg_train_state.opt_state["mu"].clone(),
                                                                  "nu": lpg_train_state.opt_state["nu"].clone()})
        new_lpg = lpg_train_state.replace(params=new_params, opt_state=opt_state, step=lpg_train_state.step + 1)
    agent_out = agent_states.replace(
        actor_state=actor.replace(params=new_actor, step=new_step),
        critic_state=critic.replace(params=new_critic, step=new_step if _static is not None else new_step.clone()),
        env_obs=new_obs, env_state=EnvState(new_state, env.max_n_objs),
        host_step=_advance_host_step(agent_states.host_step, agent_states.level.lifetime, K))
    if _static is not None:
        value_critic_states.step.add_(K + 1)
        value_out = value_critic_states
    else:
        value_out = value_critic_states.replace(step=value_critic_states.step + (K + 1))
    metrics = {
        "lpg_loss": mvec[0], "reg_lpg_loss": mvec[1], "value_loss": mvec[2],
        "lpg_agent": {"policy_l2": mvec[3], "policy_entropy": mvec[4], "critic_loss": mvec[5],
                      "critic_l2": mvec[6], "critic_entropy": mvec[7]},
        "lpg_agent_return": mvec[8],
    }
    if return_grad:
        metrics["_grad"] = grad
    if _static is not None:
        metrics["_mvec"] = mvec
    _phase("end", -1, main)
    return new_lpg, agent_out, value_out, metrics


def _advance_host_step(step, lifetime, k):
    if step is None:
        return None
    return np.minimum(step + k, np.maximum(step, lifetime)).astype(np.int32)


def _sub_level(level, sl):
    from ..util.data import Level
    return Level(level.env_params, level.lifetime[sl], level.buffer_id[sl], level.packed[sl])
```

Before: 468.7 million.

## Reuse forward segment sums in agent backward and fuse cotangent max

The agent update kernel now saves its per-run segmented gradient sums, including the trailing last-row sum, in a per-step tape buffer. When recording, it also computes the entropy-gradient segment sums at the updated parameters and stores them. The backward kernel then reads these saved sums instead of recomputing the per-token forward, entropy gradients and segment reductions. It also computes the cotangent abs-max inline, which removes the separate cotangent_max kernel, and it batches block reductions with a multi-value block_sum_n. In exchange the tape holds extra per-step buffers and the update kernel does more work when recording.

```diff
diff --git a/include/toued.h b/include/toued.h
--- a/include/toued.h
+++ b/include/toued.h
@@ -42,7 +42,8 @@
                        const float* critic_in, float* actor_out, float* critic_out,
                        const void* levels, int32_t* step, float* scalars, int n_agents,
                        int n_workers, int rollout_len, int obs_dim, float lr_actor, float lr_critic,
-                       float max_grad_norm, float agent_target_coeff, int tables_precopied, float* run_scratch,
+                       float max_grad_norm, float agent_target_coeff, int tables_precopied, float* run_sums,
+                       float* ent_sums, float policy_entropy_coeff, float target_entropy_coeff, float grad_scale,
                        void* stream);
 
 
@@ -54,12 +55,11 @@
 
 int toued_agent_backward(const int32_t* obs, const uint8_t* action, const uint16_t* sorted_tok,
                          const float* pi_hat, const float* y_hat, const float* actor_k,
-                         const float* critic_k, const float* actor_k1, const float* critic_k1,
+                         const float* critic_k, const float* grad_sums, const float* ent_sums,
                          const float* update_scalars, float* lam, float* mu, float* d_pi_hat,
-                         float* d_y_hat, int n_agents, int n_workers, int rollout_len, int obs_dim,
+                         float* d_y_hat, uint32_t* cotangent_max, int n_agents, int n_workers, int rollout_len, int obs_dim,
                          float lr_actor, float lr_critic, float max_grad_norm,
-                         float agent_target_coeff, float policy_entropy_coeff,
-                         float target_entropy_coeff, float policy_l2_coeff, float target_l2_coeff,
+                         float agent_target_coeff, float policy_l2_coeff, float target_l2_coeff,
                          float grad_scale, float* run_scratch, void* stream);
 
 int toued_transpose_wh(const float* lpg_params, float* whT, void* stream);
diff --git a/to_ued_b200/_lib.py b/to_ued_b200/_lib.py
--- a/to_ued_b200/_lib.py
+++ b/to_ued_b200/_lib.py
@@ -35,10 +35,10 @@
     "toued_sort_tokens": [_P] * 2 + [_I] * 3 + [_P],
     "toued_lpg_prepare": [_P] * 11 + [_I] * 6 + [_P],
     "toued_gru_forward": [_P] * 7 + [_I] * 5 + [_P],
-    "toued_agent_update": [_P] * 12 + [_I] * 4 + [_F] * 4 + [_I, _P, _P],
+    "toued_agent_update": [_P] * 12 + [_I] * 4 + [_F] * 4 + [_I, _P, _P] + [_F] * 3 + [_P],
     "toued_agent_scratch_floats": [_I] * 4,
     "toued_meta_loss": [_P] * 10 + [_I] * 5 + [_F] * 3 + [_I, _P],
-    "toued_agent_backward": [_P] * 14 + [_I] * 4 + [_F] * 9 + [_P, _P],
+    "toued_agent_backward": [_P] * 15 + [_I] * 4 + [_F] * 7 + [_P, _P],
     "toued_transpose_wh": [_P] * 3,
     "toued_gru_backward": [_P] * 10 + [_I] * 4 + [_P],
     "toued_lpg_wgrad_workspace_floats": [],
diff --git a/to_ued_b200/agents/lpg_agent.py b/to_ued_b200/agents/lpg_agent.py
--- a/to_ued_b200/agents/lpg_agent.py
+++ b/to_ued_b200/agents/lpg_agent.py
@@ -68,7 +68,10 @@
         self.scal_sum = torch.zeros((N, 8), dtype=f32, device=dev)
         self.step_in = torch.empty((ka, N), dtype=i32, device=dev)
         self.ep_return = torch.empty((N, W), dtype=f32, device=dev)
-        self.agent_scratch = torch.empty(_lib.lib().toued_agent_scratch_floats(N, W, L, D), dtype=f32, device=dev)
+        F = _lib.lib().toued_agent_scratch_floats(N, W, L, D)
+        self.run_sums = torch.empty((ka, F), dtype=f32, device=dev)
+        self.ent_sums = torch.empty((ka, F), dtype=f32, device=dev) if self.record else None
+        self.ent_adjoint = None
 
     def ti(self, k):
         return k if self.record else (k & 1)
@@ -146,7 +149,8 @@
     _lib.call("toued_agent_update", p(tape.obs[r]), p(tape.action[r]), p(tape.sorted_tok[r]), p(tape.pi_hat[a]),
               p(tape.y_hat[a]), p(tape.actor[t0]), p(tape.critic[t0]), p(tape.actor[t1]), p(tape.critic[t1]),
               p(levels), p(step), p(tape.scalars[a]), N, W, L, D, float(lr_actor), float(lr_critic),
-              float(max_grad_norm), float(agent_target_coeff), int(precopied), p(tape.agent_scratch), s)
+              float(max_grad_norm), float(agent_target_coeff), int(precopied), p(tape.run_sums[a]),
+              p(tape.ent_sums[a]) if tape.ent_adjoint is not None else None, *(tape.ent_adjoint or (0.0, 0.0, 0.0)), s)
     tape.scal_sum += tape.scalars[a]
     _mark("update")
 
diff --git a/to_ued_b200/csrc/agent_backward.cu b/to_ued_b200/csrc/agent_backward.cu
--- a/to_ued_b200/csrc/agent_backward.cu
+++ b/to_ued_b200/csrc/agent_backward.cu
@@ -150,19 +150,16 @@
     return f;
 }
 
-__device__ __forceinline__ void tok_grad(const TokFwd& f, float ph, const float* yh, float invT, float alpha, float* c) {
-    const float ca = invT * ph * f.q;
-#pragma unroll
-    for (int j = 0; j < 5; ++j) c[j] = ca * ((f.a == j ? 1.0f : 0.0f) - f.p[j]);
-    float mm[8], b = 0.f;
-#pragma unroll
-    for (int i = 0; i < 8; ++i) {
-        mm[i] = logf(f.y[i] + 1e-8f) - logf(yh[i] + 1e-8f) + f.y[i] / (f.y[i] + 1e-8f);
-        b = fmaf(f.y[i], mm[i], b);
-    }
-    const float cc = alpha * invT;
-#pragma unroll
-    for (int i = 0; i < 8; ++i) c[5 + i] = cc * f.y[i] * (mm[i] - b);
+__device__ __forceinline__ uint32_t abs_bits_max(uint32_t m, float v) { return max(m, __float_as_uint(v) & 0x7FFFFFFFu); }
+
+__device__ __forceinline__ void cot_max_publish(uint32_t* bits, uint32_t m) {
+    if (bits == nullptr) return;
+#pragma unroll
+    for (int o = 16; o > 0; o >>= 1) m = max(m, __shfl_xor_sync(0xffffffffu, m, o));
+    if ((threadIdx.x & 31) == 0 && m > 0u) {
+        atomicMax(bits, min(m, 0x7F800000u));
+        if (m >= 0x7F800000u) atomicOr(bits + 1, TOUED_STATUS_NONFINITE_COT);
+    }
 }
 
 __device__ __forceinline__ void load8(const float* p, float* v) {
@@ -174,14 +171,14 @@
 agent_backward_kernel(const int32_t* __restrict__ obs, const uint8_t* __restrict__ action,
                       const uint16_t* __restrict__ sorted_tok, const float* __restrict__ pi_hat,
                       const float* __restrict__ y_hat, const float* __restrict__ actor_k,
-                      const float* __restrict__ critic_k, const float* __restrict__ actor_k1,
-                      const float* __restrict__ critic_k1, const float* __restrict__ upd_scal,
-                      float* lam, float* mu, float* __restrict__ d_pi_hat, float* __restrict__ d_y_hat,
+                      const float* __restrict__ critic_k, const float* __restrict__ grad_sums, const float* __restrict__ ent_sums,
+                      const float* __restrict__ upd_scal, float* lam, float* mu, float* __restrict__ d_pi_hat,
+                      float* __restrict__ d_y_hat, uint32_t* __restrict__ cot_bits,
                       float* run_scratch, int n_agents, int W, int L, int D, float lr_a, float lr_c, float max_norm,
-                      float alpha, float b_pent, float b_yent, float b_pl2, float b_yl2, float gscale) {
+                      float alpha, float b_pl2, float b_yl2, float gscale) {
     extern __shared__ __align__(16) float rec[];
-    __shared__ float red[32];
     __shared__ float s_wlast[13];
+    __shared__ float s_lmlast[16];
     __shared__ int iscan[512];
     __shared__ unsigned char sflags[512];
     const int n = blockIdx.x, tid = threadIdx.x, T = W * L, R = n_agents * W;
@@ -190,49 +187,21 @@
     const uint16_t* st = sorted_tok + (size_t)n * T;
     const float* a0 = actor_k + (size_t)n * D * 8;
     const float* c0 = critic_k + (size_t)n * D * 8;
-    const float* a1 = actor_k1 + (size_t)n * D * 8;
-    const float* c1 = critic_k1 + (size_t)n * D * 8;
     float* lm = lam + (size_t)n * D * 8;
     float* mm = mu + (size_t)n * D * 8;
     const float invT = 1.0f / (float)T;
     const float gna = upd_scal[n * 8 + 0], gnc = upd_scal[n * 8 + 1];
     const bool keep = upd_scal[n * 8 + 2] != 0.0f;
-    float* runv = run_scratch + (size_t)n * min(T, D) * 13;
+    const int nr = min(T, D);
+    const float* gsum = grad_sums + (size_t)n * (nr + 1) * 13;
+    const float* esum = ent_sums + (size_t)n * (nr + 1) * 13;
+    float* runv = run_scratch + (size_t)n * (nr + 1) * 13;
     float* scan = rec + (size_t)T * 13;
     const SegIndex si = seg_index_build(scan + 2 * 256 * 13, iscan, st, ob, T);
 
-    float last[13];
-#pragma unroll
-    for (int j = 0; j < 13; ++j) last[j] = 0.f;
-    for (int tok = tid; tok < T; tok += 256) {
-        const TokFwd f = tok_forward(a1, c1, D, ob[tok], act[tok]);
-        float* r = rec + tok * 13;
-        {
-            float dh[5], s = 0.f;
-#pragma unroll
-            for (int j = 0; j < 5; ++j) { dh[j] = -(logf(f.p[j] + 1e-8f) + 1.0f); s = fmaf(f.p[j], dh[j], s); }
-            const float k = -b_pent * gscale * invT;
-#pragma unroll
-            for (int j = 0; j < 5; ++j) r[j] = k * f.p[j] * (dh[j] - s);
-        }
-        {
-            float dh[8], s = 0.f;
-#pragma unroll
-            for (int j = 0; j < 8; ++j) { dh[j] = -(logf(f.y[j] + 1e-8f) + 1.0f); s = fmaf(f.y[j], dh[j], s); }
-            const float k = -b_yent * gscale * invT;
-#pragma unroll
-            for (int j = 0; j < 8; ++j) r[5 + j] = k * f.y[j] * (dh[j] - s);
-        }
-#pragma unroll
-        for (int j = 0; j < 13; ++j) last[j] = fmaf(f.tf, r[j], last[j]);
-    }
-#pragma unroll
-    for (int j = 0; j < 13; ++j) last[j] = block_sum(last[j], red);
-    __syncthreads();
-    seg_reduce<13, 13>(rec, si, T, runv, scan, sflags);
-    for (int r = tid; r < si.nruns; r += 256) {
-        const int row = si.run_row[r];
-        const float* g = runv + r * 13;
+    for (int r = tid; r < si.nruns; r += 256) {
+        const int row = si.run_row[r];
+        const float* g = esum + r * 13;
 #pragma unroll
         for (int j = 0; j < 5; ++j) lm[(size_t)row * 8 + j] += g[j];
 #pragma unroll
@@ -240,47 +209,41 @@
     }
     if (tid == 0) {
 #pragma unroll
-        for (int j = 0; j < 5; ++j) lm[(size_t)(D - 1) * 8 + j] += last[j];
-#pragma unroll
-        for (int j = 0; j < 8; ++j) mm[(size_t)(D - 1) * 8 + j] += last[5 + j];
+        for (int j = 0; j < 5; ++j) lm[(size_t)(D - 1) * 8 + j] += esum[nr * 13 + j];
+#pragma unroll
+        for (int j = 0; j < 8; ++j) mm[(size_t)(D - 1) * 8 + j] += esum[nr * 13 + 5 + j];
     }
     __syncthreads();
 
     const float dir_pi = gscale * b_pl2 * 2.0f * invT;
     const float dir_y = gscale * b_yl2 * 2.0f * invT;
+    uint32_t cm = 0u;
     if (!keep) {
         for (int tok = tid; tok < T; tok += 256) {
             const int t = tok / W, w = tok - t * W;
             const size_t li = (size_t)t * R + (size_t)n * W + w;
-            d_pi_hat[li] = dir_pi * pi_hat[li];
+            const float dp = dir_pi * pi_hat[li];
+            d_pi_hat[li] = dp;
             float yh[8]; load8(y_hat + li * 8, yh);
+            float dyo[8];
+#pragma unroll
+            for (int j = 0; j < 8; ++j) { dyo[j] = dir_y * yh[j]; cm = abs_bits_max(cm, dyo[j]); }
+            cm = abs_bits_max(cm, dp);
             float4* o = reinterpret_cast<float4*>(d_y_hat + li * 8);
-            o[0] = make_float4(dir_y * yh[0], dir_y * yh[1], dir_y * yh[2], dir_y * yh[3]);
-            o[1] = make_float4(dir_y * yh[4], dir_y * yh[5], dir_y * yh[6], dir_y * yh[7]);
+            o[0] = make_float4(dyo[0], dyo[1], dyo[2], dyo[3]);
+            o[1] = make_float4(dyo[4], dyo[5], dyo[6], dyo[7]);
         }
+        cot_max_publish(cot_bits, cm);
         return;
     }
 
-#pragma unroll
-    for (int j = 0; j < 13; ++j) last[j] = 0.f;
-    for (int tok = tid; tok < T; tok += 256) {
-        const int t = tok / W, w = tok - t * W;
-        const size_t li = (size_t)t * R + (size_t)n * W + w;
-        const TokFwd f = tok_forward(a0, c0, D, ob[tok], act[tok]);
-        float yh[8]; load8(y_hat + li * 8, yh);
-        float* r = rec + tok * 13;
-        tok_grad(f, pi_hat[li], yh, invT, alpha, r);
-#pragma unroll
-        for (int j = 0; j < 13; ++j) last[j] = fmaf(f.tf, r[j], last[j]);
-    }
-#pragma unroll
-    for (int j = 0; j < 13; ++j) last[j] = block_sum(last[j], red);
-    __syncthreads();
-    seg_reduce<13, 13>(rec, si, T, runv, scan, sflags);
+    float last[13];
+#pragma unroll
+    for (int j = 0; j < 13; ++j) last[j] = gsum[nr * 13 + j];
     float dot_a = 0.f, dot_c = 0.f;
     for (int r = tid; r < si.nruns; r += 256) {
         const int row = si.run_row[r];
-        const float* g = runv + r * 13;
+        const float* g = gsum + r * 13;
         float l8[8], m8[8];
         load8(lm + (size_t)row * 8, l8); load8(mm + (size_t)row * 8, m8);
 #pragma unroll
@@ -288,7 +251,7 @@
 #pragma unroll
         for (int j = 0; j < 8; ++j) dot_c = fmaf(g[5 + j], m8[j], dot_c);
     }
-    dot_a = block_sum(dot_a, red); dot_c = block_sum(dot_c, red);
+    { float v[2] = {dot_a, dot_c}; block_sum_n<2>(v, scan); dot_a = v[0]; dot_c = v[1]; }
     float ll[8], ml[8];
     load8(lm + (size_t)(D - 1) * 8, ll); load8(mm + (size_t)(D - 1) * 8, ml);
 #pragma unroll
@@ -303,6 +266,8 @@
         for (int j = 0; j < 5; ++j) s_wlast[j] = ka * (ll[j] - pa_ * last[j]);
 #pragma unroll
         for (int j = 0; j < 8; ++j) s_wlast[5 + j] = kc * (ml[j] - pc_ * last[5 + j]);
+#pragma unroll
+        for (int j = 0; j < 8; ++j) { s_lmlast[j] = ll[j]; s_lmlast[8 + j] = ml[j]; }
     }
     __syncthreads();
     float wl[13];
@@ -311,13 +276,14 @@
 
     for (int r = tid; r < si.nruns; r += 256) {
         const int row = si.run_row[r];
-        float* g = runv + r * 13;
+        const float* g = gsum + r * 13;
+        float* wr = runv + r * 13;
         float l8[8], m8[8];
         load8(lm + (size_t)row * 8, l8); load8(mm + (size_t)row * 8, m8);
 #pragma unroll
-        for (int j = 0; j < 5; ++j) g[j] = ka * (l8[j] - pa_ * g[j]);
-#pragma unroll
-        for (int j = 0; j < 8; ++j) g[5 + j] = kc * (m8[j] - pc_ * g[5 + j]);
+        for (int j = 0; j < 5; ++j) wr[j] = ka * (l8[j] - pa_ * g[j]);
+#pragma unroll
+        for (int j = 0; j < 8; ++j) wr[5 + j] = kc * (m8[j] - pc_ * g[5 + j]);
     }
     __syncthreads();
     float hl[13];
@@ -328,54 +294,60 @@
         const int t = tok / W, w = tok - t * W;
         const size_t li = (size_t)t * R + (size_t)n * W + w;
         const TokFwd f = tok_forward(a0, c0, D, ob[tok], act[tok]);
+        const float (&p)[5] = f.p, (&y)[8] = f.y;
+        const int a = f.a;
+        const float pa = f.pa, q = f.q, tf = f.tf;
         const float ph = pi_hat[li];
         float yh[8]; load8(y_hat + li * 8, yh);
         float* r = rec + tok * 13;
         const float* wr = runv + (size_t)si.run[pos] * 13;
         float v[13];
 #pragma unroll
-        for (int j = 0; j < 13; ++j) v[j] = fmaf(f.tf, wl[j], wr[j]);
+        for (int j = 0; j < 13; ++j) v[j] = fmaf(tf, wl[j], wr[j]);
         float va = v[0], pv = 0.f;
 #pragma unroll
-        for (int j = 1; j < 5; ++j) va = (f.a == j) ? v[j] : va;
-#pragma unroll
-        for (int j = 0; j < 5; ++j) pv = fmaf(f.p[j], v[j], pv);
+        for (int j = 1; j < 5; ++j) va = (a == j) ? v[j] : va;
+#pragma unroll
+        for (int j = 0; j < 5; ++j) pv = fmaf(p[j], v[j], pv);
         const float s = va - pv;
-        d_pi_hat[li] = invT * f.q * s + dir_pi * ph;
-        const float pe = f.pa + 1e-8f;
-        const float c1_ = ph * invT * s * 1e-8f * f.pa / (pe * pe), c2_ = ph * invT * f.q;
+        const float dp = invT * q * s + dir_pi * ph;
+        d_pi_hat[li] = dp;
+        cm = abs_bits_max(cm, dp);
+        const float pe = pa + 1e-8f;
+        const float c1_ = ph * invT * s * 1e-8f * pa / (pe * pe), c2_ = ph * invT * q;
         float h[13];
 #pragma unroll
         for (int j = 0; j < 5; ++j)
-            h[j] = c1_ * ((f.a == j ? 1.0f : 0.0f) - f.p[j]) - c2_ * f.p[j] * (v[j] - pv);
+            h[j] = c1_ * ((a == j ? 1.0f : 0.0f) - p[j]) - c2_ * p[j] * (v[j] - pv);
         float m[8], mp[8], av = 0.f, b = 0.f;
 #pragma unroll
         for (int j = 0; j < 8; ++j) {
-            const float ye = f.y[j] + 1e-8f;
-            m[j] = logf(ye) - logf(yh[j] + 1e-8f) + f.y[j] / ye;
-            mp[j] = (f.y[j] + 2e-8f) / (ye * ye);
-            av = fmaf(v[5 + j], f.y[j], av);
-            b = fmaf(f.y[j], m[j], b);
+            const float ye = y[j] + 1e-8f;
+            m[j] = logf(ye) - logf(yh[j] + 1e-8f) + y[j] / ye;
+            mp[j] = (y[j] + 2e-8f) / (ye * ye);
+            av = fmaf(v[5 + j], y[j], av);
+            b = fmaf(y[j], m[j], b);
         }
         const float ca = alpha * invT;
         float dS[8], sy = 0.f, dyo[8];
 #pragma unroll
         for (int j = 0; j < 8; ++j) {
             const float vc = v[5 + j];
-            dyo[j] = ca * f.y[j] * (av - vc) / (yh[j] + 1e-8f) + dir_y * yh[j];
-            dS[j] = vc * m[j] + vc * f.y[j] * mp[j] - vc * b - av * (m[j] + f.y[j] * mp[j]);
-            sy = fmaf(f.y[j], dS[j], sy);
+            dyo[j] = ca * y[j] * (av - vc) / (yh[j] + 1e-8f) + dir_y * yh[j];
+            cm = abs_bits_max(cm, dyo[j]);
+            dS[j] = vc * m[j] + vc * y[j] * mp[j] - vc * b - av * (m[j] + y[j] * mp[j]);
+            sy = fmaf(y[j], dS[j], sy);
         }
 #pragma unroll
-        for (int j = 0; j < 8; ++j) h[5 + j] = ca * f.y[j] * (dS[j] - sy);
+        for (int j = 0; j < 8; ++j) h[5 + j] = ca * y[j] * (dS[j] - sy);
         float4* o = reinterpret_cast<float4*>(d_y_hat + li * 8);
         o[0] = make_float4(dyo[0], dyo[1], dyo[2], dyo[3]);
         o[1] = make_float4(dyo[4], dyo[5], dyo[6], dyo[7]);
 #pragma unroll
-        for (int j = 0; j < 13; ++j) { r[j] = h[j]; hl[j] = fmaf(f.tf, h[j], hl[j]); }
-    }
-#pragma unroll
-    for (int j = 0; j < 13; ++j) hl[j] = block_sum(hl[j], red);
+        for (int j = 0; j < 13; ++j) { r[j] = h[j]; hl[j] = fmaf(tf, h[j], hl[j]); }
+    }
+    cot_max_publish(cot_bits, cm);
+    block_sum_n<13>(hl, scan);
     __syncthreads();
     seg_reduce<13, 13>(rec, si, T, runv, scan, sflags);
     for (int r = tid; r < si.nruns; r += 256) {
@@ -388,33 +360,35 @@
     }
     if (tid == 0) {
 #pragma unroll
-        for (int j = 0; j < 5; ++j) lm[(size_t)(D - 1) * 8 + j] = ll[j] + hl[j];
-#pragma unroll
-        for (int j = 0; j < 8; ++j) mm[(size_t)(D - 1) * 8 + j] = ml[j] + hl[5 + j];
+        for (int j = 0; j < 5; ++j) lm[(size_t)(D - 1) * 8 + j] = s_lmlast[j] + hl[j];
+#pragma unroll
+        for (int j = 0; j < 8; ++j) mm[(size_t)(D - 1) * 8 + j] = s_lmlast[8 + j] + hl[5 + j];
     }
 }
 
 extern "C" int toued_agent_backward(const int32_t* obs, const uint8_t* action, const uint16_t* sorted_tok,
                                     const float* pi_hat, const float* y_hat, const float* actor_k,
-                                    const float* critic_k, const float* actor_k1, const float* critic_k1,
+                                    const float* critic_k, const float* grad_sums, const float* ent_sums,
                                     const float* update_scalars, float* lam, float* mu, float* d_pi_hat,
-                                    float* d_y_hat, int n_agents, int n_workers, int rollout_len, int obs_dim,
+                                    float* d_y_hat, uint32_t* cotangent_max, int n_agents, int n_workers, int rollout_len, int obs_dim,
                                     float lr_actor, float lr_critic, float max_grad_norm,
-                                    float agent_target_coeff, float policy_entropy_coeff,
-                                    float target_entropy_coeff, float policy_l2_coeff, float target_l2_coeff,
+                                    float agent_target_coeff, float policy_l2_coeff, float target_l2_coeff,
                                     float grad_scale, float* run_scratch, void* stream) {
     const int T = n_workers * rollout_len;
     TOUED_CHECK(n_agents > 0 && T > 0, "toued_agent_backward: empty problem");
     TOUED_CHECK(run_scratch != nullptr, "toued_agent_backward: run_scratch (toued_agent_scratch_floats) is required");
+    TOUED_CHECK(grad_sums != nullptr && ent_sums != nullptr,
+                "toued_agent_backward: the update's run sums (run_sums, ent_sums of toued_agent_update) are required");
     const size_t smem = sizeof(float) * ((size_t)T * 13 + 2 * 256 * 13) + seg_index_bytes(T);
     TOUED_CHECK(smem <= 200 * 1024, "toued_agent_backward: W*L=%d too large for shared memory", T);
     TOUED_CUDA(cudaFuncSetAttribute(agent_backward_kernel, cudaFuncAttributeMaxDynamicSharedMemorySize, (int)smem));
     TOUED_CUDA(cudaFuncSetAttribute(agent_backward_kernel, cudaFuncAttributePreferredSharedMemoryCarveout, 100));
     cudaStream_t st = (cudaStream_t)stream;
+    if (cotangent_max) TOUED_CUDA(cudaMemsetAsync(cotangent_max, 0, sizeof(uint32_t), st));
     agent_backward_kernel<<<n_agents, 256, smem, st>>>(
-        obs, action, sorted_tok, pi_hat, y_hat, actor_k, critic_k, actor_k1, critic_k1, update_scalars, lam, mu,
-        d_pi_hat, d_y_hat, run_scratch, n_agents, n_workers, rollout_len, obs_dim, lr_actor, lr_critic, max_grad_norm,
-        agent_target_coeff, policy_entropy_coeff, target_entropy_coeff, policy_l2_coeff, target_l2_coeff, grad_scale);
+        obs, action, sorted_tok, pi_hat, y_hat, actor_k, critic_k, grad_sums, ent_sums, update_scalars, lam, mu,
+        d_pi_hat, d_y_hat, cotangent_max, run_scratch, n_agents, n_workers, rollout_len, obs_dim, lr_actor, lr_critic, max_grad_norm,
+        agent_target_coeff, policy_l2_coeff, target_l2_coeff, grad_scale);
     TOUED_LAUNCH_CHECK();
     return 0;
 }
diff --git a/to_ued_b200/csrc/agent_update.cu b/to_ued_b200/csrc/agent_update.cu
--- a/to_ued_b200/csrc/agent_update.cu
+++ b/to_ued_b200/csrc/agent_update.cu
@@ -10,14 +10,15 @@
                     const float* __restrict__ y_hat, const float* __restrict__ actor_in,
                     const float* __restrict__ critic_in, float* actor_out, float* critic_out,
                     const LevelRec* __restrict__ levels, int32_t* __restrict__ step,
-                    float* __restrict__ scal, float* run_scratch, int n_agents, int W, int L, int D,
-                    float lr_a, float lr_c, float max_norm, float alpha, int tables_precopied) {
+                    float* __restrict__ scal, float* run_sums, float* ent_sums, int n_agents, int W, int L, int D,
+                    float lr_a, float lr_c, float max_norm, float alpha, int tables_precopied, float b_pent,
+                    float b_yent, float gscale) {
     extern __shared__ __align__(16) float smc[];
-    __shared__ float red[32];
     __shared__ int iscan[512];
     __shared__ unsigned char sflags[512];
     const int n = blockIdx.x, tid = threadIdx.x, T = W * L, R = n_agents * W;
-    float* runv = run_scratch + (size_t)n * min(T, D) * 13;
+    const int nr = min(T, D);
+    float* runv = run_sums + (size_t)n * (nr + 1) * 13;
     float* scan = smc + (size_t)T * AU_C;
     void* idxmem = scan + 2 * 256 * 13;
     const int32_t* ob = obs + (size_t)n * (L + 1) * W;
@@ -77,12 +78,22 @@
         for (int j = 0; j < 13; ++j) last[j] = fmaf(tf, rec[j], last[j]);
         m_kl += kl; m_pi2 = fmaf(ph, ph, m_pi2); m_y2 += y2;
     }
-#pragma unroll
-    for (int j = 0; j < 13; ++j) last[j] = block_sum(last[j], red);
-    m_kl = block_sum(m_kl, red); m_pi2 = block_sum(m_pi2, red); m_y2 = block_sum(m_y2, red);
+    {
+        float v[16];
+#pragma unroll
+        for (int j = 0; j < 13; ++j) v[j] = last[j];
+        v[13] = m_kl; v[14] = m_pi2; v[15] = m_y2;
+        block_sum_n<16>(v, scan);
+#pragma unroll
+        for (int j = 0; j < 13; ++j) last[j] = v[j];
+        m_kl = v[13]; m_pi2 = v[14]; m_y2 = v[15];
+    }
     __syncthreads();
 
     seg_reduce<13, AU_C>(smc, si, T, runv, scan, sflags);
+    if (tid == 0)
+#pragma unroll
+        for (int j = 0; j < 13; ++j) runv[nr * 13 + j] = last[j];
     float na = 0.f, nc = 0.f;
     for (int r = tid; r < si.nruns; r += 256) {
         const float* g = runv + r * 13;
@@ -91,7 +102,7 @@
 #pragma unroll
         for (int j = 5; j < 13; ++j) nc = fmaf(g[j], g[j], nc);
     }
-    na = block_sum(na, red); nc = block_sum(nc, red);
+    { float v[2] = {na, nc}; block_sum_n<2>(v, scan); na = v[0]; nc = v[1]; }
 #pragma unroll
     for (int j = 0; j < 5; ++j) na = fmaf(last[j], last[j], na);
 #pragma unroll
@@ -120,7 +131,11 @@
     }
     __syncthreads();
 
+    const bool ent = ent_sums != nullptr;
     float ea = 0.f, ec = 0.f;
+    float elast[13];
+#pragma unroll
+    for (int j = 0; j < 13; ++j) elast[j] = 0.f;
     for (int tok = tid; tok < T; tok += 256) {
         const int32_t o = ob[tok];
         float z[5], p[5], zy[8], y[8];
@@ -132,8 +147,49 @@
         for (int j = 0; j < 5; ++j) { const float q = p[j] + 1e-8f; ea -= q * logf(q); }
 #pragma unroll
         for (int j = 0; j < 8; ++j) { const float q = y[j] + 1e-8f; ec -= q * logf(q); }
-    }
-    ea = block_sum(ea, red); ec = block_sum(ec, red);
+        if (ent) {
+            float* r = smc + tok * AU_C;
+            {
+                float dh[5], s = 0.f;
+#pragma unroll
+                for (int j = 0; j < 5; ++j) { dh[j] = -(logf(p[j] + 1e-8f) + 1.0f); s = fmaf(p[j], dh[j], s); }
+                const float k = -b_pent * gscale * invT;
+#pragma unroll
+                for (int j = 0; j < 5; ++j) r[j] = k * p[j] * (dh[j] - s);
+            }
+            {
+                float dh[8], s = 0.f;
+#pragma unroll
+                for (int j = 0; j < 8; ++j) { dh[j] = -(logf(y[j] + 1e-8f) + 1.0f); s = fmaf(y[j], dh[j], s); }
+                const float k = -b_yent * gscale * invT;
+#pragma unroll
+                for (int j = 0; j < 8; ++j) r[5 + j] = k * y[j] * (dh[j] - s);
+            }
+            const float tf = 0.001f * (float)ob_time(o);
+#pragma unroll
+            for (int j = 0; j < 13; ++j) elast[j] = fmaf(tf, r[j], elast[j]);
+        }
+    }
+    if (ent) {
+        float* env = ent_sums + (size_t)n * (nr + 1) * 13;
+        float v[15];
+#pragma unroll
+        for (int j = 0; j < 13; ++j) v[j] = elast[j];
+        v[13] = ea; v[14] = ec;
+        block_sum_n<15>(v, scan);
+#pragma unroll
+        for (int j = 0; j < 13; ++j) elast[j] = v[j];
+        ea = v[13]; ec = v[14];
+        __syncthreads();
+        seg_reduce<13, AU_C>(smc, si, T, env, scan, sflags);
+        if (tid == 0)
+#pragma unroll
+            for (int j = 0; j < 13; ++j) env[nr * 13 + j] = elast[j];
+    } else {
+        float v[2] = {ea, ec};
+        block_sum_n<2>(v, scan);
+        ea = v[0]; ec = v[1];
+    }
     if (tid == 0) {
         float* s = scal + (size_t)n * 8;
         s[0] = gna; s[1] = gnc; s[2] = keep ? 1.0f : 0.0f;
@@ -155,7 +211,8 @@
                                   const void* levels, int32_t* step, float* scalars, int n_agents,
                                   int n_workers, int rollout_len, int obs_dim, float lr_actor,
                                   float lr_critic, float max_grad_norm, float agent_target_coeff, int tables_precopied,
-                                  float* run_scratch, void* stream) {
+                                  float* run_sums, float* ent_sums, float policy_entropy_coeff,
+                                  float target_entropy_coeff, float grad_scale, void* stream) {
     const int T = n_workers * rollout_len;
     const size_t smem = agent_smem_bytes(T, obs_dim);
     TOUED_CHECK(n_agents > 0 && T > 0, "toued_agent_update: empty problem");
@@ -163,18 +220,19 @@
     TOUED_CHECK(actor_in != actor_out && critic_in != critic_out, "toued_agent_update: in-place update not supported");
     TOUED_CUDA(cudaFuncSetAttribute(agent_update_kernel, cudaFuncAttributeMaxDynamicSharedMemorySize, (int)smem));
     TOUED_CUDA(cudaFuncSetAttribute(agent_update_kernel, cudaFuncAttributePreferredSharedMemoryCarveout, 100));
-    TOUED_CHECK(run_scratch != nullptr, "toued_agent_update: run_scratch (toued_agent_scratch_floats) is required");
+    TOUED_CHECK(run_sums != nullptr, "toued_agent_update: run_sums (toued_agent_scratch_floats) is required");
     cudaStream_t st = (cudaStream_t)stream;
     agent_update_kernel<<<n_agents, 256, smem, st>>>(
         obs, action, sorted_tok, pi_hat, y_hat, actor_in, critic_in, actor_out, critic_out,
-        (const LevelRec*)levels, step, scalars, run_scratch, n_agents, n_workers, rollout_len, obs_dim,
-        lr_actor, lr_critic, max_grad_norm, agent_target_coeff, tables_precopied);
+        (const LevelRec*)levels, step, scalars, run_sums, ent_sums, n_agents, n_workers, rollout_len, obs_dim,
+        lr_actor, lr_critic, max_grad_norm, agent_target_coeff, tables_precopied, policy_entropy_coeff,
+        target_entropy_coeff, grad_scale);
     TOUED_LAUNCH_CHECK();
     return 0;
 }
 
 extern "C" int toued_agent_scratch_floats(int n_agents, int n_workers, int rollout_len, int obs_dim) {
     const long long T = (long long)n_workers * rollout_len;
-    const long long n = 13ll * (T < obs_dim ? T : obs_dim) * n_agents;
+    const long long n = 13ll * ((T < obs_dim ? T : obs_dim) + 1) * n_agents;
     return n < (1ll << 31) ? (int)n : -1;
 }
diff --git a/to_ued_b200/csrc/lpg_common.cuh b/to_ued_b200/csrc/lpg_common.cuh
--- a/to_ued_b200/csrc/lpg_common.cuh
+++ b/to_ued_b200/csrc/lpg_common.cuh
@@ -85,3 +85,24 @@
     for (int o = 16; o > 0; o >>= 1) t += __shfl_xor_sync(0xffffffffu, t, o);
     return t;
 }
+
+template <int N>
+__device__ __forceinline__ void block_sum_n(float (&v)[N], float* red) {
+#pragma unroll
+    for (int j = 0; j < N; ++j)
+#pragma unroll
+        for (int o = 16; o > 0; o >>= 1) v[j] += __shfl_xor_sync(0xffffffffu, v[j], o);
+    const int lane = threadIdx.x & 31, warp = threadIdx.x >> 5, nw = (blockDim.x + 31) >> 5;
+    __syncthreads();
+    if (lane == 0)
+#pragma unroll
+        for (int j = 0; j < N; ++j) red[j * 32 + warp] = v[j];
+    __syncthreads();
+#pragma unroll
+    for (int j = 0; j < N; ++j) {
+        float t = (lane < nw) ? red[j * 32 + lane] : 0.0f;
+#pragma unroll
+        for (int o = 16; o > 0; o >>= 1) t += __shfl_xor_sync(0xffffffffu, t, o);
+        v[j] = t;
+    }
+}
diff --git a/to_ued_b200/meta/train.py b/to_ued_b200/meta/train.py
--- a/to_ued_b200/meta/train.py
+++ b/to_ued_b200/meta/train.py
@@ -186,6 +186,7 @@
                              _sub_level(agent_states.level, sl), agent_states.env_obs[sl],
                              EnvState(agent_states.env_state.packed[sl], env.max_n_objs))
             levels = sub.level.packed
+            tape.ent_adjoint = (float(bK[0]), float(bK[1]), float(gscale))
             gens[mb] = (train_lpg_agent_steps(r_train[sl], lpg_train_state, sub, rollout_manager, K,
                                               lpg_hypers.agent_target_coeff, tape=tape), sl, levels)
             next(gens[mb][0])
@@ -248,10 +249,10 @@
     def _agent_backward(ws, tape, k, buf, s):
         _lib.call("toued_agent_backward", p(tape.obs[k]), p(tape.action[k]), p(tape.sorted_tok[k]),
                   p(tape.pi_hat[k]), p(tape.y_hat[k]), p(tape.actor[k]), p(tape.critic[k]),
-                  p(tape.actor[k + 1]), p(tape.critic[k + 1]), p(tape.scalars[k]), p(ws.lam), p(ws.mu),
-                  p(ws.d_pi_hat2[buf]), p(ws.d_y_hat2[buf]), nb, W, L, D, float(actor.learning_rate),
+                  p(tape.run_sums[k]), p(tape.ent_sums[k]), p(tape.scalars[k]), p(ws.lam), p(ws.mu),
+                  p(ws.d_pi_hat2[buf]), p(ws.d_y_hat2[buf]), p(ws.cotmax[k]) if tc else None, nb, W, L, D, float(actor.learning_rate),
                   float(critic.learning_rate), float(actor.max_grad_norm),
-                  float(lpg_hypers.agent_target_coeff), *[float(b) for b in bK], float(gscale), p(ws.ab_scratch), s)
+                  float(lpg_hypers.agent_target_coeff), *[float(b) for b in bK[2:]], float(gscale), p(ws.ab_scratch), s)
 
     def backward_step(mb, k):
         slot = mb % S
@@ -277,8 +278,6 @@
             if k + 2 <= K - 1:
                 st.wait_event(ev["wg"][k + 2])
             _agent_backward(ws, tape, k, buf, _lib.stream_ptr())
-            _lib.call("toued_cotangent_max", p(ws.d_pi_hat2[buf]), p(ws.d_y_hat2[buf]), nb, W, L, p(ws.cotmax[k]),
-                      _lib.stream_ptr())
             ev["ab"][k].record(st)
         with torch.cuda.stream(streams[slot]):
             st = streams[slot]
```

New measurement: 480.9 million, median of 6. 1.03x the previous value.
